# scroll-tech/scroll-prover

Hardware: AMD Instinct MI355X
Metric: BN254 MSM G1-adds/sec at k=26 (higher is better)
Workload: dtype u32 (9x29-bit limbs of 254-bit Montgomery integers; v_mad_u64_u32); 1 GPU; BN254 G1 Pippenger MSM, 2^26 uniform random scalars x synthetic SRS points, inputs resident in HBM; point-range shards over 1 GPU(s), RCCL all-gather of 96-B partials; log_n=26, window_bits=22, windows=12, parallelism=point-range x1, one rank per GPU, srs_window_tables=True

## Files before the change

### scroll-prover_amd/csrc/fp29.hpp

```cpp
#pragma once
#include "fp.hpp"

namespace zk {

struct fe29_t { uint32_t l[9]; };
constexpr uint32_t M29 = (1u << 29) - 1;

struct Fq29P {
  static constexpr uint32_t INV = 0x4866389u;
  ZK_HD static constexpr uint32_t mod(int i) { constexpr uint32_t m[9] = {0x187cfd47u, 0x10460b6u, 0x1c72a34fu, 0x2d522d0u, 0x1585d978u, 0x2db40c0u, 0xa6e141u, 0xe5c2634u, 0x30644eu}; return m[i]; }
  ZK_HD static constexpr uint32_t one(int i) { constexpr uint32_t m[9] = {0x157ccc21u, 0x141c2758u, 0x185230d3u, 0x14c0419u, 0xaa36fb9u, 0x1d4240ceu, 0x11d54c07u, 0x52ac7a8u, 0xdc836u}; return m[i]; }
  ZK_HD static constexpr uint32_t r256(int i) { constexpr uint32_t m[9] = {0x58f0d9du, 0x1aea1c6eu, 0x11c2cf74u, 0x11d651ebu, 0x1462c0a7u, 0x11b7bc3cu, 0x1cbd99bau, 0x183340fbu, 0xe0a77u}; return m[i]; }
  ZK_HD static constexpr uint32_t fat29_4p(int i) { constexpr uint32_t m[9] = {0x21f3f51cu, 0x241182dau, 0x31ca8d3bu, 0x2b548b42u, 0x361765dfu, 0x2b6d0301u, 0x229b8503u, 0x397098cfu, 0xc19138u}; return m[i]; }
  ZK_HD static constexpr uint32_t fat30_8p(int i) { constexpr uint32_t m[9] = {0x43e7ea38u, 0x482305b4u, 0x43951a76u, 0x56a91685u, 0x4c2ecbbeu, 0x56da0603u, 0x45370a06u, 0x52e1319eu, 0x1832271u}; return m[i]; }
  ZK_HD static constexpr uint32_t fat30_16p(int i) { constexpr uint32_t m[9] = {0x47cfd470u, 0x50460b6au, 0x472a34eeu, 0x4d522d0cu, 0x585d977fu, 0x4db40c08u, 0x4a6e140fu, 0x45c2633eu, 0x30644e5u}; return m[i]; }
};
struct Fr29P {
  static constexpr uint32_t INV = 0xfffffffu;
  ZK_HD static constexpr uint32_t mod(int i) { constexpr uint32_t m[9] = {0x10000001u, 0x1f0fac9fu, 0xe5c2450u, 0x7d090f3u, 0x1585d283u, 0x2db40c0u, 0xa6e141u, 0xe5c2634u, 0x30644eu}; return m[i]; }
  ZK_HD static constexpr uint32_t one(int i) { constexpr uint32_t m[9] = {0xfffff57u, 0x1ea70ab4u, 0x52c068bu, 0x17504f49u, 0xaa8075bu, 0x1d4240ceu, 0x11d54c07u, 0x52ac7a8u, 0xdc836u}; return m[i]; }
  ZK_HD static constexpr uint32_t r256(int i) { constexpr uint32_t m[9] = {0xffffffbu, 0x4b1a0e2u, 0x18334a6bu, 0x18ed2b3eu, 0x1462e36fu, 0x11b7bc3cu, 0x1cbd99bau, 0x183340fbu, 0xe0a77u}; return m[i]; }
  ZK_HD static constexpr uint32_t fat29_4p(int i) { constexpr uint32_t m[9] = {0x20000004u, 0x3c3eb27du, 0x39709142u, 0x3f4243ccu, 0x36174a0bu, 0x2b6d0301u, 0x229b8503u, 0x397098cfu, 0xc19138u}; return m[i]; }
  ZK_HD static constexpr uint32_t fat30_8p(int i) { constexpr uint32_t m[9] = {0x40000008u, 0x587d64fau, 0x52e12285u, 0x5e848799u, 0x4c2e9417u, 0x56da0603u, 0x45370a06u, 0x52e1319eu, 0x1832271u}; return m[i]; }
  ZK_HD static constexpr uint32_t fat30_16p(int i) { constexpr uint32_t m[9] = {0x40000010u, 0x50fac9f6u, 0x45c2450du, 0x5d090f35u, 0x585d2831u, 0x4db40c08u, 0x4a6e140fu, 0x45c2633eu, 0x30644e5u}; return m[i]; }
};

#if defined(__HIP_DEVICE_COMPILE__)
#include "fp29_asm_gen.inc"
#endif

template <class P> struct Fp29 {
  ZK_HD static fe29_t zero() { fe29_t r; for (int i = 0; i < 9; i++) r.l[i] = 0; return r; }
  ZK_HD static fe29_t one() { fe29_t r; for (int i = 0; i < 9; i++) r.l[i] = P::one(i); return r; }

  ZK_HD static fe29_t mul(const fe29_t &a, const fe29_t &b) {
    uint64_t acc = 0; uint32_t m[9]; fe29_t r;
#pragma unroll
    for (int k = 0; k < 9; k++) {
#pragma unroll
      for (int i = 0; i <= k; i++) acc += (uint64_t)a.l[i] * b.l[k - i];
#pragma unroll
      for (int i = 0; i < k; i++) acc += (uint64_t)m[i] * P::mod(k - i);
      m[k] = ((uint32_t)acc * P::INV) & M29;
      acc += (uint64_t)m[k] * P::mod(0);
      acc >>= 29;
    }
#pragma unroll
    for (int k = 9; k < 17; k++) {
#pragma unroll
      for (int i = k - 8; i < 9; i++) acc += (uint64_t)a.l[i] * b.l[k - i];
#pragma unroll
      for (int i = k - 8; i < 9; i++) acc += (uint64_t)m[i] * P::mod(k - i);
      r.l[k - 9] = (uint32_t)acc & M29;
      acc >>= 29;
    }
    r.l[8] = (uint32_t)acc;
    return r;
  }
  ZK_HD static fe29_t sqr(const fe29_t &a) {
    uint64_t acc = 0; uint32_t m[9]; fe29_t r;
    uint32_t a2[9];
#pragma unroll
    for (int i = 0; i < 9; i++) a2[i] = a.l[i] << 1;
#pragma unroll
    for (int k = 0; k < 9; k++) {
#pragma unroll
      for (int i = 0; 2 * i < k; i++) acc += (uint64_t)a.l[i] * a2[k - i];
      if ((k & 1) == 0) acc += (uint64_t)a.l[k / 2] * a.l[k / 2];
#pragma unroll
      for (int i = 0; i < k; i++) acc += (uint64_t)m[i] * P::mod(k - i);
      m[k] = ((uint32_t)acc * P::INV) & M29;
      acc += (uint64_t)m[k] * P::mod(0);
      acc >>= 29;
    }
#pragma unroll
    for (int k = 9; k < 17; k++) {
#pragma unroll
      for (int i = k - 8; 2 * i < k; i++) acc += (uint64_t)a.l[i] * a2[k - i];
      if ((k & 1) == 0) acc += (uint64_t)a.l[k / 2] * a.l[k / 2];
#pragma unroll
      for (int i = k - 8; i < 9; i++) acc += (uint64_t)m[i] * P::mod(k - i);
      r.l[k - 9] = (uint32_t)acc & M29;
      acc >>= 29;
    }
    r.l[8] = (uint32_t)acc;
    return r;
  }
  ZK_HD static fe29_t mul_sub(const fe29_t &a, const fe29_t &b, const fe29_t &c, const fe29_t &d) {
    int64_t acc = 0; uint32_t m[9]; fe29_t r;
    int32_t nc[9];
#pragma unroll
    for (int i = 0; i < 9; i++) nc[i] = -(int32_t)c.l[i];
#pragma unroll
    for (int k = 0; k < 9; k++) {
#pragma unroll
      for (int i = 0; i <= k; i++) { acc += (int64_t)(int32_t)a.l[i] * (int32_t)b.l[k - i]; acc += (int64_t)nc[i] * (int32_t)d.l[k - i]; }
#pragma unroll
      for (int i = 0; i < k; i++) acc += (int64_t)(int32_t)m[i] * (int32_t)P::mod(k - i);
      m[k] = ((uint32_t)acc * P::INV) & M29;
      acc += (int64_t)(int32_t)m[k] * (int32_t)P::mod(0);
      acc >>= 29;
    }
#pragma unroll
    for (int k = 9; k < 17; k++) {
#pragma unroll
      for (int i = k - 8; i < 9; i++) { acc += (int64_t)(int32_t)a.l[i] * (int32_t)b.l[k - i]; acc += (int64_t)nc[i] * (int32_t)d.l[k - i]; }
#pragma unroll
      for (int i = k - 8; i < 9; i++) acc += (int64_t)(int32_t)m[i] * (int32_t)P::mod(k - i);
      r.l[k - 9] = ((uint32_t)acc & M29) + P::mod(k - 9);
      acc >>= 29;
    }
    r.l[8] = (uint32_t)((int32_t)acc + (int32_t)P::mod(8));
    return r;
  }
  ZK_HD static fe29_t mul_c(const fe29_t &a, const fe29_t &b) {
#if defined(__HIP_DEVICE_COMPILE__)
    uint64_t acc = 0, co; uint32_t m[9]; fe29_t r;
    ZK_FP29_MUL_COLUMNS
    (void)co;
    return r;
#else
    return mul(a, b);
#endif
  }
  ZK_HD static fe29_t sqr_c(const fe29_t &a) {
#if defined(__HIP_DEVICE_COMPILE__)
    uint64_t acc = 0, co; uint32_t m[9]; fe29_t r;
    uint32_t a2[9];
#pragma unroll
    for (int i = 0; i < 9; i++) a2[i] = a.l[i] << 1;
    ZK_FP29_SQR_COLUMNS
    (void)co;
    return r;
#else
    return sqr(a);
#endif
  }
  ZK_HD static fe29_t mul_sub_c(const fe29_t &a, const fe29_t &b, const fe29_t &c, const fe29_t &d) {
#if defined(__HIP_DEVICE_COMPILE__)
    int64_t acc = 0; uint64_t co; uint32_t m[9]; fe29_t r;
    int32_t nc[9];
#pragma unroll
    for (int i = 0; i < 9; i++) nc[i] = -(int32_t)c.l[i];
    ZK_FP29_MULSUB_COLUMNS
    (void)co;
    return r;
#else
    return mul_sub(a, b, c, d);
#endif
  }
  ZK_HD static fe29_t carry(const fe29_t &a) {
    fe29_t r; r.l[0] = a.l[0] & M29;
#pragma unroll
    for (int i = 1; i < 8; i++) r.l[i] = (a.l[i] & M29) + (a.l[i - 1] >> 29);
    r.l[8] = a.l[8] + (a.l[7] >> 29);
    return r;
  }
  ZK_HD static fe29_t add(const fe29_t &a, const fe29_t &b) { fe29_t r; for (int i = 0; i < 9; i++) r.l[i] = a.l[i] + b.l[i]; return r; }
  ZK_HD static fe29_t sub4(const fe29_t &a, const fe29_t &b) {
    fe29_t r;
#pragma unroll
    for (int i = 0; i < 9; i++) r.l[i] = a.l[i] + P::fat29_4p(i) - b.l[i];
    return carry(r);
  }
  ZK_HD static fe29_t sub4_lazy(const fe29_t &a, const fe29_t &b) {
    fe29_t r;
#pragma unroll
    for (int i = 0; i < 9; i++) r.l[i] = a.l[i] + P::fat29_4p(i) - b.l[i];
    return r;
  }
  ZK_HD static fe29_t sub8(const fe29_t &a, const fe29_t &b) {
    fe29_t r;
#pragma unroll
    for (int i = 0; i < 9; i++) r.l[i] = a.l[i] + P::fat30_8p(i) - b.l[i];
    return carry(r);
  }
  ZK_HD static fe29_t sub4_8(const fe29_t &a, const fe29_t &b, const fe29_t &c) {
    fe29_t r;
#pragma unroll
    for (int i = 0; i < 9; i++) r.l[i] = a.l[i] + (P::fat29_4p(i) + P::fat30_8p(i)) - b.l[i] - c.l[i];
    return carry(r);
  }
  ZK_HD static fe29_t sub16(const fe29_t &a, const fe29_t &b) {
    fe29_t r;
#pragma unroll
    for (int i = 0; i < 9; i++) r.l[i] = a.l[i] + P::fat30_16p(i) - b.l[i];
    return carry(r);
  }
  ZK_HD static fe29_t dbl(const fe29_t &a) { fe29_t r; for (int i = 0; i < 9; i++) r.l[i] = a.l[i] << 1; return r; }

  ZK_HD static fe29_t normalise(const fe29_t &a) {
    fe29_t r; uint32_t c = 0;
#pragma unroll
    for (int i = 0; i < 8; i++) { uint32_t v = a.l[i] + c; r.l[i] = v & M29; c = v >> 29; }
    r.l[8] = a.l[8] + c;
    return r;
  }
  ZK_HD static fe29_t cond_sub_p(const fe29_t &a) {
    fe29_t d; uint32_t borrow = 0;
#pragma unroll
    for (int i = 0; i < 9; i++) { uint32_t v = a.l[i] - P::mod(i) - borrow; borrow = v >> 31; d.l[i] = (i < 8) ? (v & M29) : v; }
    fe29_t r;
#pragma unroll
    for (int i = 0; i < 9; i++) r.l[i] = borrow ? a.l[i] : d.l[i];
    return r;
  }
  ZK_HD static fe29_t reduce_small(const fe29_t &v) {
    const uint32_t q = (uint32_t)(((uint64_t)(v.l[8] >> 12) * 0x15291u) >> 26);
    fe29_t r; int64_t c = 0;
#pragma unroll
    for (int i = 0; i < 9; i++) { c += (int64_t)v.l[i] - (int64_t)((uint64_t)q * P::mod(i)); r.l[i] = (i < 8) ? ((uint32_t)c & M29) : (uint32_t)c; c >>= 29; }
    return r;
  }
  ZK_HD static bool is_zero_tight(const fe29_t &a) {
    if (a.l[0] != 0 && a.l[0] != P::mod(0)) return false;
    uint32_t z = 0, q = 0;
#pragma unroll
    for (int i = 0; i < 9; i++) { z |= a.l[i]; q |= a.l[i] ^ P::mod(i); }
    return z == 0 || q == 0;
  }
  ZK_HD static fe29_t from_sat(const fe_t &s) {
    fe29_t r;
    r.l[0] = (s.l[0] << 5) & M29;
#pragma unroll
    for (int i = 1; i < 9; i++) {
      const int bit = 29 * i - 5, w = bit >> 5, sh = bit & 31;
      uint32_t v = s.l[w] >> sh;
      if (sh > 3 && w + 1 < 8) v |= s.l[w + 1] << (32 - sh);
      r.l[i] = v & M29;
    }
    return r;
  }
  ZK_HD static fe29_t from_sat_plain(const fe_t &s) {
    fe29_t r;
#pragma unroll
    for (int i = 0; i < 9; i++) {
      const int bit = 29 * i, w = bit >> 5, sh = bit & 31;
      uint32_t v = s.l[w] >> sh;
      if (sh > 3 && w + 1 < 8) v |= s.l[w + 1] << (32 - sh);
      r.l[i] = v & M29;
    }
    return r;
  }
  ZK_HD static fe_t to_sat_plain(const fe29_t &a) {
    fe_t s;
#pragma unroll
    for (int w = 0; w < 8; w++) {
      const int bit = 32 * w, i = bit / 29, sh = bit - 29 * i;
      uint64_t v = (uint64_t)a.l[i] >> sh;
      v |= (uint64_t)a.l[i + 1] << (29 - sh);
      if (i + 2 < 9) v |= (uint64_t)a.l[i + 2] << (58 - sh);
      s.l[w] = (uint32_t)v;
    }
    return s;
  }
  ZK_HD static fe_t to_sat(const fe29_t &a) {
    fe29_t c; for (int i = 0; i < 9; i++) c.l[i] = P::r256(i);
    fe29_t t = cond_sub_p(normalise(mul(a, c)));
    return to_sat_plain(t);
  }
};

using Fq29 = Fp29<Fq29P>;
using Fr29 = Fp29<Fr29P>;

}
```

### scroll-prover_amd/csrc/g1_29.hpp

```cpp
#pragma once
#include "fp29.hpp"
#include "g1.hpp"

namespace zk {

struct g1_xyzz29_t { fe29_t x, y, zz, zzz; };

ZK_HD g1_xyzz29_t g1_xyzz29_identity() { g1_xyzz29_t r; r.x = Fq29::zero(); r.y = Fq29::zero(); r.zz = Fq29::zero(); r.zzz = Fq29::zero(); return r; }
ZK_HD bool g1_xyzz29_is_identity(const g1_xyzz29_t &p) { uint32_t o = 0; for (int i = 0; i < 9; i++) o |= p.zz.l[i]; return o == 0; }

ZK_HD fe29_t fq29_neg_loaded(const fe29_t &y) {
  constexpr uint32_t c[9] = {0x3f3f51c0u, 0x21182dafu, 0x3ca8d3c1u, 0x3548b437u, 0x21765e04u, 0x36d0302au, 0x29b85044u, 0x37098d00u, 0xc19139bu};
  fe29_t r;
#pragma unroll
  for (int i = 0; i < 9; i++) r.l[i] = c[i] - y.l[i];
  return r;
}

ZK_HD g1_xyzz29_t g1_xyzz29_dbl_affine(const fe29_t &xt, const fe29_t &yt) {
  const fe29_t U = Fq29::dbl(yt);
  const fe29_t V = Fq29::sqr_c(U), W = Fq29::mul_c(U, V), S = Fq29::mul_c(xt, V);
  const fe29_t xx = Fq29::sqr_c(xt);
  const fe29_t M = Fq29::carry(Fq29::add(Fq29::dbl(xx), xx));
  g1_xyzz29_t r;
  r.x = Fq29::sub8(Fq29::sqr_c(M), Fq29::dbl(S));
  const fe29_t t = Fq29::sub16(S, r.x);
  r.y = Fq29::sub4(Fq29::mul_c(M, t), Fq29::mul_c(W, yt));
  r.zz = V; r.zzz = W;
  return r;
}

ZK_HD bool g1_affine_is_identity_x(const g1_affine_t &q) { return Fq::is_zero(q.x); }
ZK_HD fe29_t fq29_negx(const fe29_t &x) { return Fq29::sub16(Fq29::zero(), x); }
ZK_HD void g1_xyzz29_negx_to_plain(g1_xyzz29_t &acc) { if (!g1_xyzz29_is_identity(acc)) acc.x = fq29_negx(acc.x); }

ZK_HD void g1_xyzz29_madd_core(g1_xyzz29_t &acc, const fe29_t &x2, const fe29_t &y2, bool y2_needs_normalise);
ZK_HD void g1_xyzz29_madd(g1_xyzz29_t &acc, const g1_affine_t &q, bool negate) {
  if (g1_affine_is_identity_x(q)) return;
  const fe29_t x2 = Fq29::from_sat(q.x);
  fe29_t y2 = Fq29::from_sat(q.y);
  if (negate) y2 = fq29_neg_loaded(y2);
  g1_xyzz29_madd_core(acc, x2, y2, negate);
}
ZK_HD void g1_xyzz29_madd_core(g1_xyzz29_t &acc, const fe29_t &x2, const fe29_t &y2, bool y2_needs_normalise) {
  if (g1_xyzz29_is_identity(acc)) {
    acc.x = Fq29::reduce_small(x2); acc.y = Fq29::reduce_small(y2_needs_normalise ? Fq29::normalise(y2) : y2);
    acc.x = Fq29::sub4(Fq29::zero(), acc.x);
    acc.zz = Fq29::one(); acc.zzz = Fq29::one();
    return;
  }
  const fe29_t U2 = Fq29::mul_c(x2, acc.zz), S2 = Fq29::mul_c(y2, acc.zzz);
  const fe29_t Pd = Fq29::add(U2, acc.x);
  const fe29_t Rd = Fq29::sub8(S2, acc.y);
  const fe29_t PP = Fq29::sqr_c(Pd);
  const fe29_t ZZ3 = Fq29::mul_c(acc.zz, PP);
  if (Fq29::is_zero_tight(ZZ3)) {
    const fe29_t one = Fq29::one();
    if (Fq29::is_zero_tight(Fq29::mul(Rd, one))) { acc = g1_xyzz29_dbl_affine(Fq29::mul(x2, one), Fq29::mul(y2, one)); acc.x = fq29_negx(acc.x); }
    else acc = g1_xyzz29_identity();
    return;
  }
  const fe29_t PPP = Fq29::mul_c(Pd, PP);
  const fe29_t Qn = Fq29::mul_c(acc.x, PP);
  const fe29_t xn3 = Fq29::sub4_8(PPP, Fq29::sqr_c(Rd), Fq29::dbl(Qn));
  const fe29_t T = Fq29::sub4_lazy(xn3, Qn);
  const fe29_t Y3 = Fq29::mul_sub_c(Rd, T, acc.y, PPP);
  acc.x = xn3; acc.y = Y3; acc.zz = ZZ3; acc.zzz = Fq29::mul_c(acc.zzz, PPP);
}

ZK_HD g1_xyzz29_t g1_xyzz29_dbl(const g1_xyzz29_t &a) {
  if (g1_xyzz29_is_identity(a)) return a;
  const fe29_t xt = Fq29::reduce_small(Fq29::normalise(a.x));
  const fe29_t yc = Fq29::carry(a.y);
  const fe29_t U = Fq29::dbl(yc);
  const fe29_t V = Fq29::sqr_c(U), W = Fq29::mul_c(U, V), S = Fq29::mul_c(xt, V);
  const fe29_t xx = Fq29::sqr_c(xt);
  const fe29_t M = Fq29::carry(Fq29::add(Fq29::dbl(xx), xx));
  g1_xyzz29_t r;
  r.x = Fq29::sub8(Fq29::sqr_c(M), Fq29::dbl(S));
  const fe29_t t = Fq29::sub16(S, r.x);
  r.y = Fq29::sub4(Fq29::mul_c(M, t), Fq29::mul_c(W, yc));
  r.zz = Fq29::mul_c(V, a.zz); r.zzz = Fq29::mul_c(W, a.zzz);
  return r;
}

ZK_HD void g1_xyzz29_add(g1_xyzz29_t &acc, const g1_xyzz29_t &q) {
  if (g1_xyzz29_is_identity(q)) return;
  if (g1_xyzz29_is_identity(acc)) { acc = q; return; }
  const fe29_t U1 = Fq29::mul_c(acc.x, q.zz), S1 = Fq29::mul_c(acc.y, q.zzz);
  const fe29_t U2 = Fq29::mul_c(q.x, acc.zz), S2 = Fq29::mul_c(q.y, acc.zzz);
  const fe29_t Pd = Fq29::sub4(U2, U1);
  const fe29_t Rd = Fq29::sub4(S2, S1);
  const fe29_t PP = Fq29::sqr_c(Pd);
  const fe29_t ZZt = Fq29::mul_c(acc.zz, PP);
  if (Fq29::is_zero_tight(ZZt)) {
    if (Fq29::is_zero_tight(Fq29::mul_c(Rd, Fq29::one()))) acc = g1_xyzz29_dbl(acc);
    else acc = g1_xyzz29_identity();
    return;
  }
  const fe29_t PPP = Fq29::mul_c(Pd, PP);
  const fe29_t Q = Fq29::mul_c(U1, PP);
  const fe29_t X3 = Fq29::sub4_8(Fq29::sqr_c(Rd), PPP, Fq29::dbl(Q));
  const fe29_t Y3 = Fq29::mul_sub_c(Rd, Fq29::sub16(Q, X3), S1, PPP);
  acc.x = X3; acc.y = Y3;
  acc.zz = Fq29::mul_c(ZZt, q.zz); acc.zzz = Fq29::mul_c(Fq29::mul_c(acc.zzz, PPP), q.zzz);
}

ZK_HD g1_xyzz_t g1_xyzz29_to_sat(const g1_xyzz29_t &a) {
  g1_xyzz_t r;
  if (g1_xyzz29_is_identity(a)) return g1_xyzz_identity();
  r.x = Fq29::to_sat(a.x); r.y = Fq29::to_sat(a.y); r.zz = Fq29::to_sat(a.zz); r.zzz = Fq29::to_sat(a.zzz);
  return r;
}

}
```

### scroll-prover_amd/csrc/lib_common.hpp

```cpp
#pragma once
#include <hip/hip_runtime.h>
#include <stdio.h>
#include <stdlib.h>
#include <string.h>
#include <algorithm>
#include <atomic>
#include <chrono>
#include <map>
#include <memory>
#include <mutex>
#include <string>
#include <thread>
#include <condition_variable>
#include <unordered_map>
#include <vector>

#include "../../include/mi355zk.h"
#include "fp.hpp"
#include "g1.hpp"
#include "g1_29.hpp"
#include "ntt_types.hpp"
#include "ws_layout.hpp"
#include "knobs.hpp"

namespace mi355 {
using namespace zk;
using mi355zk::WsLayout;

extern thread_local std::string g_err;
int fail(int code, const std::string &msg);

#define HIPCHK(expr)                                                                                                     \
  do {                                                                                                                   \
    hipError_t _e = (expr);                                                                                              \
    if (_e != hipSuccess) {                                                                                              \
      char _b[512]; snprintf(_b, sizeof _b, "%s failed: %s (%s:%d)", #expr, hipGetErrorString(_e), __FILE__, __LINE__);  \
      (void)hipGetLastError();                                                                                           \
      return ::mi355::fail(_e == hipErrorOutOfMemory ? MI355_EOOM : MI355_EHIP, _b);                                     \
    }                                                                                                                    \
  } while (0)
#define CHK(expr) do { int _r = (expr); if (_r != MI355_OK) return _r; } while (0)

struct Shard { int slot = 0; uint64_t lo = 0, n = 0; g1_affine_t *dev = nullptr; bool owned = false; };
void free_shards(std::vector<Shard> &sh);
struct SrsMem { std::vector<Shard> sh; ~SrsMem() { free_shards(sh); } };
struct SrsTables { std::vector<g1_affine_t *> pre; std::vector<uint64_t> stride; std::vector<int> slot; int c = 0, w = 0; ~SrsTables(); };
struct Srs { uint64_t n = 0; std::shared_ptr<SrsMem> mem; std::shared_ptr<SrsTables> tab; };
struct Buf { void *p = nullptr; size_t cap = 0; };
struct NttPlan {
  uint32_t log_n = 0, levels = 0, log_m[3] = {0, 0, 0};
  uint32_t split[2] = {0, 0};
  uint32_t direct2[2] = {0, 0};
  std::map<std::string, Tw29> scaled;
  struct CosetTw { Tw29 in, s2d; };
  std::map<std::string, CosetTw> coset;
  Tw29 tw29_m[3] = {}, tw29_s_lo[2] = {}, tw29_s_hi[2] = {};
  std::vector<void *> owned;
};
struct Prof { double ms = 0; uint64_t launches = 0; };

struct MsmSlot { int id = 0; hipEvent_t sorted = nullptr, acc_done = nullptr, red_done = nullptr; bool used = false; };

struct Span { std::string name; hipEvent_t a, b; };
struct Ctx : mi355zk::Knobs {
  bool inited = false;
  int slot = 0;
  int device = -1;
  hipDeviceProp_t prop;
  hipStream_t own_stream = nullptr, stream = nullptr;
  hipStream_t aux_stream[2] = {nullptr, nullptr};
  hipStream_t copy_stream = nullptr;
  MsmSlot msm_slot[2];
  hipEvent_t ev_fork = nullptr;
  hipEvent_t ev_xchg = nullptr;
  hipEvent_t ev_xchg2 = nullptr;
  hipEvent_t ev_copy[4] = {};
  hipEvent_t ev_up[8] = {}; uint32_t up_next = 0;
  hipEvent_t ev_up_fork = nullptr;
  void *comm = nullptr;
  std::vector<const fe_t *> polys_stage;
  uint32_t msm_chunk_min_log = 23;
  int last_chunks = 1;
  std::map<std::string, Buf> ws;
  std::map<std::string, NttPlan> ntt_plans;
  g1_affine_t *fixed_base_table = nullptr;
  bool profiling = false;
  std::vector<Span> spans;
  std::map<std::string, Prof> prof;
  int last_c = 0, last_w = 0; uint64_t last_entries = 0; bool last_shared = false; int last_host_slices = 1;
};
enum : unsigned { SYNC_COMPUTE = 1, SYNC_AUX = 2, SYNC_COPY = 4 };
struct CtxStream { hipStream_t *s; unsigned kind; };
inline std::vector<CtxStream> ctx_streams(Ctx &c) { return {{&c.own_stream, SYNC_COMPUTE}, {&c.aux_stream[0], SYNC_AUX}, {&c.aux_stream[1], SYNC_AUX}, {&c.copy_stream, SYNC_COPY}}; }
inline std::vector<hipEvent_t *> ctx_events(Ctx &c) {
  std::vector<hipEvent_t *> v = {&c.ev_fork, &c.ev_xchg, &c.ev_xchg2, &c.ev_up_fork};
  for (auto &m : c.msm_slot) { v.push_back(&m.sorted); v.push_back(&m.acc_done); v.push_back(&m.red_done); }
  for (auto &e : c.ev_copy) v.push_back(&e);
  for (auto &e : c.ev_up) v.push_back(&e);
  return v;
}
hipError_t sync_streams(Ctx &c, unsigned which);

constexpr int MAX_DEV = 16;
extern std::mutex g_ctx_mu[MAX_DEV];
extern std::mutex g_upload_mu[MAX_DEV];
extern Ctx g_ctx[MAX_DEV];
extern int g_ndev;
extern bool g_dup_devices;
extern bool g_peer_ok[MAX_DEV][MAX_DEV];
extern mi355zk::ProcessKnobs g_proc;
extern thread_local Ctx *g_cur;
#define g (*::mi355::g_cur)
extern std::unordered_map<uint64_t, Srs> &g_srs;
extern uint64_t g_next_handle;
extern int g_last_devices; extern const char *g_last_exchange;

struct DevGuard {
  std::unique_lock<std::mutex> lk;
  explicit DevGuard(int slot) : lk(g_ctx_mu[slot]) {}
};
struct AllGuard {
  std::unique_lock<std::mutex> lk[MAX_DEV];
  AllGuard() { for (int i = 0; i < MAX_DEV; i++) lk[i] = std::unique_lock<std::mutex>(g_ctx_mu[i]); }
};
struct MsmGuard {
  std::unique_lock<std::mutex> lk[MAX_DEV];
  MsmGuard() { lk[0] = std::unique_lock<std::mutex>(g_ctx_mu[0]); for (int i = 1; i < g_ndev && i < MAX_DEV; i++) lk[i] = std::unique_lock<std::mutex>(g_ctx_mu[i]); }
};

struct PoolBlock {
  void *p = nullptr; int slot = 0;
  PoolBlock() = default;
  PoolBlock(const PoolBlock &) = delete; PoolBlock &operator=(const PoolBlock &) = delete;
  ~PoolBlock() { if (p) (void)mi355_buf_free(p); }
  int alloc(uint64_t bytes, int slot_) { slot = slot_; return mi355_buf_alloc(bytes, slot_, &p); }
  char *at(uint64_t off) const { return (char *)p + off; }
  int upload(uint64_t off, const void *src_host, uint64_t bytes);
};

struct MsmOpts { bool normalise = true; int force_c = 0; bool no_tables = false; };
extern thread_local MsmOpts t_opts;

inline void use_ctx(int slot) { g_cur = &g_ctx[slot]; }
int bind_ctx(int slot);
int need_init(int slot = 0);
inline int PoolBlock::upload(uint64_t off, const void *src_host, uint64_t bytes) { CHK(mi355_buf_upload(at(off), src_host, bytes)); return need_init(slot); }

struct CallTrace {
  const char *what; uint64_t n; double bytes_per_unit; std::chrono::steady_clock::time_point t0;
  CallTrace(const char *w, uint64_t n_, double bpu) : what(w), n(n_), bytes_per_unit(bpu), t0(std::chrono::steady_clock::now()) {}
  void done(const char *extra = "") {
    if (!g.trace) return;
    (void)hipStreamSynchronize(g.stream);
    const double ms = std::chrono::duration<double, std::milli>(std::chrono::steady_clock::now() - t0).count();
    fprintf(stderr, "[mi355zk] %s n=%llu %.3f ms %.2f M units/s %.1f GB/s algorithmic%s\n", what, (unsigned long long)n, ms, n / ms / 1e3, n * bytes_per_unit / ms / 1e6, extra);
  }
};

int ws_get(const char *role, size_t bytes, void **out);
int dev_malloc(void **out, size_t bytes, const char *what);

struct Scope {
  bool on; hipEvent_t a = nullptr, b = nullptr; std::string name; hipStream_t st;
  Scope(const char *n, hipStream_t s = nullptr) : on(g.profiling), name(n), st(s ? s : g.stream) { if (on) { (void)hipEventCreate(&a); (void)hipEventCreate(&b); (void)hipEventRecord(a, st); } }
  void close() { if (on) { (void)hipEventRecord(b, st); g.spans.push_back({name, a, b}); on = false; } }
  ~Scope() { close(); }
};
void resolve_spans();
inline int finish_async() { if (g.profiling) resolve_spans(); return MI355_OK; }

inline uint32_t ceil_div(uint64_t a, uint64_t b) { return (uint32_t)((a + b - 1) / b); }
inline uint32_t log2_ceil(uint64_t n) { uint32_t l = 0; while ((1ull << l) < n) l++; return l; }

struct Roctx { int state = 0; int (*push)(const char *) = nullptr; int (*pop)() = nullptr; };
extern Roctx g_roctx;
void roctx_bind();
struct ApiRange {
  bool on;
  explicit ApiRange(const char *name) : on(false) { if (g_roctx.state == 0) roctx_bind(); if (g_roctx.state == 2) { g_roctx.push(name); on = true; } }
  ~ApiRange() { if (on) g_roctx.pop(); }
};
template <class F> int guarded(F body, const char *who = __builtin_FUNCTION()) {
  ApiRange range(who);
  try { return body(); }
  catch (const std::bad_alloc &) { return fail(MI355_EOOM, "host allocation failed"); }
  catch (const std::exception &e) { return fail(MI355_EHIP, std::string("unexpected host exception: ") + e.what()); }
  catch (...) { return fail(MI355_EHIP, "unexpected host exception"); }
}

struct Rccl {
  void *lib = nullptr;
  int (*CommInitAll)(void **, int, const int *) = nullptr;
  int (*CommDestroy)(void *) = nullptr;
  int (*AllGather)(const void *, void *, size_t, int, void *, hipStream_t) = nullptr;
  int (*GroupStart)() = nullptr;
  int (*GroupEnd)() = nullptr;
  const char *(*GetErrorString)(int) = nullptr;
};
extern Rccl g_rccl;
int rccl_fail(const char *what, int rc);

std::vector<Shard> plan_shards(uint64_t n);
int srs_find(uint64_t handle, Srs **out, const char *who);
uint64_t srs_insert(const Srs &s);
int srs_alloc(SrsMem &mem, uint64_t n);
int srs_scatter_from_primary(SrsMem &mem, const g1_affine_t *src_dev, uint64_t n, bool alias_shard0);
int srs_gather_to_primary(const Srs &sr, uint64_t n, const g1_affine_t **out);

int slot_of(const void *dev_ptr, bool touch = true);
int buf_check_range(const void *dev_ptr, uint64_t bytes, const char *who);
int common_slot(std::initializer_list<const void *> ptrs, int *slot_out, const char *who);
int common_slot(const void *const *ptrs, size_t count, bool touch, int *slot_out, const char *who);
int pick_replica_slot();

int msm_tu_init_device();
int ntt_tu_init_device();
int aux_tu_init_device();
int launch_pow_table(fe_t *out, const fe_t &base, uint64_t step, uint32_t count);
int launch_g1_decompress(const void *bytes_dev, void *affine_out_dev, uint64_t n, uint64_t base, unsigned long long *err_dev);
bool g2_decode_host(const uint8_t in[64], void *g2affine_out);
constexpr int MSM_SCALAR_BITS = 255, MSM_MAX_C = 24;
double msm_cost(uint64_t n, int c, bool shared);

inline int check_ntt_args(const void *data, uint32_t log_n, const void *omega) {
  if (!data || !omega) return fail(MI355_EBADARG, "ntt: null pointer");
  if (log_n > 28) return fail(MI355_EBADARG, "ntt: log_n > 28");
  return MI355_OK;
}
struct NttHostArgs { uint32_t log_n; const void *omega; const void *divisor; };
inline int with_host_io(void *data_host, size_t in_bytes, size_t out_bytes, size_t dev_bytes, const char *role, int (*body)(void *dev, void *ud), void *ud) {
  void *dev; CHK(ws_get(role, dev_bytes, &dev));
  HIPCHK(hipMemcpyAsync(dev, data_host, in_bytes, hipMemcpyHostToDevice, g.stream));
  CHK(body(dev, ud));
  HIPCHK(hipMemcpyAsync(data_host, dev, out_bytes, hipMemcpyDeviceToHost, g.stream));
  HIPCHK(hipStreamSynchronize(g.stream));
  resolve_spans();
  return MI355_OK;
}

}
```

### scroll-prover_amd/csrc/lib_msm.hip

```cpp
#define ZK_FRSCAN_DEVICE_ONLY 1
#include "msm.hpp"
#define ZK_G2_DEVICE_ONLY 1
#include "msm_g2.hpp"
#include "msm_seg.hpp"
#include "lib_common.hpp"

namespace mi355 {

static_assert(sizeof(fe_t) == 32 && sizeof(g1_affine_t) == 64 && sizeof(g1_jac_t) == 96, "ABI element sizes");
static_assert(sizeof(g1_xyzz_t) == 128 && sizeof(g1_xyzz29_t) == 144, "device record sizes (workspace layout, 16-byte vector accesses)");

int msm_tu_init_device() {
  HIPCHK(hipFuncSetAttribute((const void *)k_sort_l1_scatter_split<24>, hipFuncAttributeMaxDynamicSharedMemorySize, 160 * 1024));
  HIPCHK(hipFuncSetAttribute((const void *)k_sort_l1_scatter_split<16>, hipFuncAttributeMaxDynamicSharedMemorySize, 160 * 1024));
  HIPCHK(hipFuncSetAttribute((const void *)k_sort_l1_scatter_split<8>, hipFuncAttributeMaxDynamicSharedMemorySize, 160 * 1024));
  HIPCHK(hipFuncSetAttribute((const void *)k_sort_l2_scatter_split<16>, hipFuncAttributeMaxDynamicSharedMemorySize, 160 * 1024));
  HIPCHK(hipFuncSetAttribute((const void *)k_sort_l2_scatter_split<8>, hipFuncAttributeMaxDynamicSharedMemorySize, 160 * 1024));
  return MI355_OK;
}

double msm_cost(uint64_t n, int c, bool shared) { const double W = (MSM_SCALAR_BITS + c - 1) / c, nb = (double)(1ull << (c - 1)); return 1.18 * W * (double)n + 8.2 * nb * (shared ? 1.0 : W) + (shared ? 0.0 : 3.0e7); }

int choose_c(uint64_t n) {
  if (t_opts.force_c) return t_opts.force_c;
  double best = 1e300; int best_c = 8;
  for (int c = 4; c <= (int)g_proc.msm_auto_max_c; c++) {
    const double W = (MSM_SCALAR_BITS + c - 1) / c, nb = (double)(1ull << (c - 1));
    if (W * nb * sizeof(g1_xyzz29_t) > 6.0e9) continue;
    const double cost = msm_cost(n, c, false);
    if (cost < best) { best = cost; best_c = c; }
  }
  return best_c;
}

struct PreTable { const g1_affine_t *table = nullptr; uint64_t row_stride = 0; int c = 0, w = 0; };
const PreTable *pre_advance(const PreTable *pre, uint64_t lo, PreTable &store) {
  if (!pre) return nullptr;
  store = *pre; if (store.table) store.table += lo;
  return &store;
}

struct MsmShape { bool shared; uint32_t c, W, fb, cb_bits, regions; uint64_t emax, nbuckets; };
int msm_shape(uint64_t n, uint32_t M, const PreTable *pre, MsmShape &o, const MsmShape *forced = nullptr) {
  if (forced) { o.c = forced->c; o.shared = forced->shared; }
  else {
    o.c = (uint32_t)choose_c(n);
    o.shared = pre && pre->table && !t_opts.force_c && !t_opts.no_tables && msm_cost(n, pre->c, true) <= msm_cost(n, (int)o.c, false) && ((uint64_t)pre->w << log2_ceil(n)) < (1ull << 31);
    if (o.shared) o.c = (uint32_t)pre->c;
  }
  o.W = (MSM_SCALAR_BITS + o.c - 1) / o.c;
  o.emax = (uint64_t)M * n * o.W;
  const uint32_t kb = o.c - 1; uint32_t fb = kb < g.sort_fb ? kb : g.sort_fb; if (kb - fb > 11) fb = kb - 11;
  o.fb = fb; o.cb_bits = kb - fb;
  const uint64_t sets = (uint64_t)M * (o.shared ? 1 : o.W);
  o.nbuckets = sets << kb;
  const uint64_t regions = sets << o.cb_bits; o.regions = (uint32_t)std::min<uint64_t>(regions, 0xffffffffu);
  if (o.emax >= (1ull << 32)) return fail(MI355_EBADARG, "msm: n * windows must be < 2^32");
  if (o.nbuckets >= (1ull << 31)) return fail(MI355_EBADARG, "msm: too many buckets (split the batch)");
  if (regions * 4 > 48 * 1024) return fail(MI355_EBADARG, "msm: batch too large for the coarse histogram (split the batch)");
  if (o.fb > 12 || (1u << o.cb_bits) > SORT_MAX_BINS) return fail(MI355_EBADARG, "msm: window bits out of range for the sorter");
  return MI355_OK;
}

template <class G> bool msm_batch_must_split(uint64_t n, uint32_t M, const PreTable *pre) {
  MsmShape sh;
  return msm_shape(n, M, pre, sh) != MI355_OK || sh.emax > (1ull << 29) || sh.nbuckets * sizeof(typename G::rec_t) > (8ull << 30);
}

struct Roles {
  const char *prefix; std::string sfx;
  template <class T> int get(const char *name, size_t bytes, T *&ptr) const { return ws_get((std::string(prefix) + name + sfx).c_str(), bytes, (void **)&ptr); }
};

int msm_stage_polys(const fe_t *const *polys_host, uint32_t M, const Roles &ws, hipStream_t s, PolyPtrs &inl, const fe_t **&polys_dev) {
  if (M <= 8) { for (uint32_t m = 0; m < M; m++) inl.p[m] = polys_host[m]; return MI355_OK; }
  CHK(ws.get("polys", (size_t)M * sizeof(void *), polys_dev));
  g.polys_stage.assign(polys_host, polys_host + M);
  HIPCHK(hipMemcpyAsync(polys_dev, g.polys_stage.data(), (size_t)M * sizeof(void *), hipMemcpyHostToDevice, s));
  HIPCHK(hipStreamSynchronize(s));
  return MI355_OK;
}

struct AccPlan { uint32_t seg, blocks, tn; };
AccPlan msm_acc_plan(uint64_t emax) {
  const uint64_t want_threads = (uint64_t)g.prop.multiProcessorCount * 256 * g.seg_factor;
  uint64_t seg = (emax + want_threads - 1) / want_threads; if (seg < 16) seg = 16; if (seg > 4096) seg = 4096;
  const uint32_t blocks = ceil_div(ceil_div(emax, seg), 256);
  return {(uint32_t)seg, blocks, blocks * 256};
}
uint32_t msm_seg_arg(uint32_t seg, uint32_t fill_pct) { return seg | (std::min(g.seg_min, seg) << 13) | ((fill_pct / 2) << 26); }
MsmPlan msm_plan(const MsmShape &sh, uint64_t n, uint32_t M, uint32_t seg) {
  MsmPlan P; P.n = (uint32_t)n; P.c = sh.c; P.windows = sh.W; P.nb = 1u << (sh.c - 1); P.seg = seg; P.batch = M;
  return P;
}

template <class G, class F> void with_lanes(bool quad, F &&launch) {
  if constexpr (G::QUAD) { if (quad) { launch(std::integral_constant<int, 4>{}); return; } }
  launch(std::integral_constant<int, 1>{});
}

template <class G> int msm_segfix_levels(const int32_t *part_id, const typename G::rec_t *part, uint32_t tn, typename G::rec_t *buckets, hipStream_t s, const Roles &ws) {
  using rec_t = typename G::rec_t;
  uint32_t N = 2 * tn; const uint32_t waves1 = ceil_div(N, 64);
  const size_t cap = (size_t)2 * waves1 + (size_t)waves1 / 8 + 512;
  int32_t *lv_ids; rec_t *lv_recs;
  CHK(ws.get("segfix_ids", cap * 4, lv_ids)); CHK(ws.get("segfix_recs", cap * sizeof(rec_t), lv_recs));
  const int32_t *cur_ids = part_id; const rec_t *cur_recs = part; size_t used = 0;
  while (N > 64) {
    const uint32_t waves = ceil_div(N, 64);
    hipLaunchKernelGGL(k_msm_segfix<G>, dim3(ceil_div(N, 256)), dim3(256), 0, s, cur_ids, cur_recs, N, buckets, lv_ids + used, lv_recs + used, 0);
    cur_ids = lv_ids + used; cur_recs = lv_recs + used; used += (size_t)2 * waves; N = 2 * waves;
  }
  hipLaunchKernelGGL(k_msm_segfix<G>, dim3(1), dim3(64), 0, s, cur_ids, cur_recs, N, buckets, (int32_t *)nullptr, (rec_t *)nullptr, 1);
  return MI355_OK;
}

template <class G> int msm_reduce_tail(const MsmShape &sh, uint32_t M, const typename G::rec_t *buckets, typename G::out_t *out_dev, bool normalise, hipStream_t s, const Roles &ws) {
  using rec_t = typename G::rec_t;
  const uint32_t nb = 1u << (sh.c - 1), wpp = sh.shared ? 1 : sh.W, sets = M * wpp;
  uint32_t chunk = 64; while (chunk > nb) chunk >>= 1;
  while (chunk > g.reduce_min_chunk && (uint64_t)(nb / chunk) * sets < g.reduce_chains) chunk >>= 1;
  const uint32_t chunks_per_set = nb / chunk, nchunks = chunks_per_set * sets;
  rec_t *chunk_out, *tree_a, *tree_b, *window_sums;
  CHK(ws.get("chunk_out", (size_t)nchunks * sizeof(rec_t), chunk_out));
  { const size_t lvl = (size_t)ceil_div(chunks_per_set, 64 * TREE_PER_THREAD) * sets + 1;
    CHK(ws.get("tree_a", lvl * sizeof(rec_t), tree_a)); CHK(ws.get("tree_b", lvl * sizeof(rec_t), tree_b)); }
  CHK(ws.get("window_sums", (size_t)sets * sizeof(rec_t), window_sums));
  with_lanes<G>(nchunks <= g.tail_coop_max && (g.tail_coop_mask & 2u), [&](auto q) {
    constexpr int Q = decltype(q)::value;
    hipLaunchKernelGGL((k_msm_bucket_reduce<G, Q>), dim3(ceil_div((uint64_t)nchunks * Q, 128)), dim3(128), 0, s, buckets, chunk_out, nb, sets, chunk);
  });
  const rec_t *cur = chunk_out; uint32_t cnt = chunks_per_set; rec_t *bufs[2] = {tree_a, tree_b}; int which = 0;
  while (true) {
    const bool coop = G::QUAD && (uint64_t)cnt * sets <= g.tail_coop_max && (g.tail_coop_mask & 4u);
    const uint32_t outn = ceil_div(cnt, (coop ? 64u : 256u) * TREE_PER_THREAD);
    rec_t *dst = outn == 1 ? window_sums : bufs[which];
    with_lanes<G>(coop, [&](auto q) { hipLaunchKernelGGL((k_msm_tree_sum<G, decltype(q)::value>), dim3(outn, sets), dim3(256), 0, s, cur, cnt, dst, outn); });
    if (outn == 1) break;
    cur = dst; cnt = outn; which ^= 1;
  }
  with_lanes<G>(g.tail_coop_max && (g.tail_coop_mask & 8u), [&](auto q) {
    hipLaunchKernelGGL((k_msm_final<G, decltype(q)::value>), dim3(M), dim3(64), 0, s, (const rec_t *)window_sums, wpp, sh.shared ? 0u : sh.c, out_dev, normalise ? 1 : 0);
  });
  HIPCHK(hipGetLastError());
  return MI355_OK;
}

int msm_sort_stage(const PolyPtrs &inl, const fe_t *const *polys_dev, uint32_t M, uint64_t n, const MsmShape &sh, const MsmPlan &P, uint32_t *offsets, uint32_t *sorted,
                   hipStream_t s, bool g2 = false) {
  const bool shared = sh.shared;
  const uint64_t emax = sh.emax;
  const uint32_t nbuckets = (uint32_t)sh.nbuckets;
  SortPlan S; S.n = P.n; S.windows = M * P.windows; S.wpp = P.windows; S.nb = P.nb;
  S.fb = sh.fb; S.cb_bits = sh.cb_bits;
  S.shared = shared ? 1 : 0; S.nshift = log2_ceil(n);
  S.regions = sh.regions;
  S.t1 = g.sort_t1;
  if (g.sort_split == 1 && S.t1 == 16384 && (1u << S.cb_bits) <= 1024 && emax >= (1ull << 24)) S.t1 = 24576;
  S.t2 = g.sort_t2 ? g.sort_t2 : (emax >= (1ull << 27) && S.fb <= 11 ? 16384 : 8192);
  const uint32_t tiles1 = ceil_div(n, S.t1), l2_tiles_max = ceil_div(emax, S.t2) + S.regions + 8;
  const uint32_t vwindows = M * P.windows;

  uint32_t *enc, *hist, *cursor, *scan_sums, *coarse_hist, *coarse_off, *coarse_cursor, *tile_start;
  CHK(ws_get("msm.digits", emax * 4, (void **)&enc));
  uint32_t *pairs_lo = nullptr; uint16_t *pairs_hi = nullptr;
  CHK(ws_get("msm.pairs_lo", emax * 4 + 64, (void **)&pairs_lo)); CHK(ws_get("msm.pairs_hi", emax * 2 + 64, (void **)&pairs_hi));
  CHK(ws_get("msm.hist", ((size_t)nbuckets + 1) * 4, (void **)&hist));
  CHK(ws_get("msm.cursor", ((size_t)nbuckets + 1) * 4, (void **)&cursor));
  CHK(ws_get("msm.coarse_hist", ((size_t)S.regions + 1) * 4, (void **)&coarse_hist));
  CHK(ws_get("msm.coarse_off", ((size_t)S.regions + 1) * 4, (void **)&coarse_off));
  CHK(ws_get("msm.coarse_cursor", ((size_t)S.regions + 1) * 4, (void **)&coarse_cursor));
  CHK(ws_get("msm.tile_start", ((size_t)S.regions + 1) * 4, (void **)&tile_start));
  const uint32_t scan_n = nbuckets + 1, scan_blocks = ceil_div(scan_n, SCAN_BLOCK * SCAN_ITEMS);
  const uint32_t cscan_n = S.regions + 1, cscan_blocks = ceil_div(cscan_n, SCAN_BLOCK * SCAN_ITEMS);
  CHK(ws_get("msm.scan_sums", (size_t)(scan_blocks + cscan_blocks) * 4, (void **)&scan_sums));
  const int grid_stream = g.prop.multiProcessorCount * 8;
  {
    Scope sc(g2 ? "msm_g2_digits" : "msm_digits", s);
    HIPCHK(hipMemsetAsync(coarse_hist, 0, ((size_t)S.regions + 1) * 4, s));
    const dim3 dgrid(grid_stream / M > 0 ? grid_stream / M : 1, M);
    if (g2) hipLaunchKernelGGL(k_msm_digits<false>, dgrid, dim3(256), (size_t)S.regions * 4, s, inl, polys_dev, enc, P, coarse_hist, S.fb, S.cb_bits, S.shared);
    else hipLaunchKernelGGL(k_msm_digits<true>, dgrid, dim3(256), (size_t)S.regions * 4, s, inl, polys_dev, enc, P, coarse_hist, S.fb, S.cb_bits, S.shared);
  }
  {
    Scope sc(g2 ? "msm_g2_sort" : "msm_sort", s);
    HIPCHK(hipMemsetAsync(hist, 0, ((size_t)nbuckets + 1) * 4, s));
    hipLaunchKernelGGL(k_scan_partial, dim3(cscan_blocks), dim3(SCAN_BLOCK), 0, s, coarse_hist, scan_sums + scan_blocks, cscan_n);
    hipLaunchKernelGGL(k_scan_block_sums, dim3(1), dim3(SCAN_BLOCK), 0, s, scan_sums + scan_blocks, cscan_blocks);
    hipLaunchKernelGGL(k_scan_final, dim3(cscan_blocks), dim3(SCAN_BLOCK), 0, s, coarse_hist, scan_sums + scan_blocks, coarse_off, coarse_cursor, cscan_n);
    {
      Scope s1(g2 ? "g2_sort_l1" : "sort_l1", s);
      const uint32_t CBp = ((1u << S.cb_bits) + 1) & ~1u;
      const size_t lds1 = (size_t)(3 * CBp + 32 + SORT_SPLIT_TMAX) * 4 + (size_t)S.t1 * 6;
      if (S.t1 == 24576) hipLaunchKernelGGL(k_sort_l1_scatter_split<24>, dim3(tiles1 * vwindows), dim3(1024), lds1, s, enc, coarse_cursor, pairs_lo, pairs_hi, S);
      else if (S.t1 == 16384) hipLaunchKernelGGL(k_sort_l1_scatter_split<16>, dim3(tiles1 * vwindows), dim3(1024), lds1, s, enc, coarse_cursor, pairs_lo, pairs_hi, S);
      else hipLaunchKernelGGL(k_sort_l1_scatter_split<8>, dim3(tiles1 * vwindows), dim3(1024), lds1, s, enc, coarse_cursor, pairs_lo, pairs_hi, S);
    }
    hipLaunchKernelGGL(k_sort_tile_prefix, dim3(1), dim3(SCAN_BLOCK), 0, s, coarse_off, tile_start, S);
    { Scope s2(g2 ? "g2_sort_hist" : "sort_hist", s);
    hipLaunchKernelGGL(k_sort_l2_hist_split, dim3(l2_tiles_max), dim3(256), 0, s, (const uint16_t *)pairs_hi, coarse_off, tile_start, hist, S); }
    hipLaunchKernelGGL(k_scan_partial, dim3(scan_blocks), dim3(SCAN_BLOCK), 0, s, hist, scan_sums, scan_n);
    hipLaunchKernelGGL(k_scan_block_sums, dim3(1), dim3(SCAN_BLOCK), 0, s, scan_sums, scan_blocks);
    hipLaunchKernelGGL(k_scan_final, dim3(scan_blocks), dim3(SCAN_BLOCK), 0, s, hist, scan_sums, offsets, cursor, scan_n);
    {
      Scope s3(g2 ? "g2_sort_l2" : "sort_l2", s);
      const size_t lds2 = (size_t)(3 * (1u << S.fb) + 32) * 4 + (size_t)S.t2 * 6;
      if (S.t2 == 8192) hipLaunchKernelGGL(k_sort_l2_scatter_split<8>, dim3(l2_tiles_max), dim3(1024), lds2, s, (const uint32_t *)pairs_lo, (const uint16_t *)pairs_hi, coarse_off, tile_start, cursor, sorted, S);
      else hipLaunchKernelGGL(k_sort_l2_scatter_split<16>, dim3(l2_tiles_max), dim3(1024), lds2, s, (const uint32_t *)pairs_lo, (const uint16_t *)pairs_hi, coarse_off, tile_start, cursor, sorted, S);
    }
  }
  return MI355_OK;
}

struct MsmStreams { hipStream_t a, b, c; };

int msm_enqueue(const g1_affine_t *bases, const PolyPtrs &inl, const fe_t *const *polys_dev, uint32_t M, uint64_t n, g1_jac_t *out_dev, const PreTable *pre, MsmSlot &slot,
                const MsmStreams &st, bool normalise, const MsmShape *forced = nullptr, uint32_t set_index = 0, uint32_t set_count = 1, bool skip_tail = false) {
  const bool piped = st.a != st.b;
  const Roles ws{G1Ops::ROLE, slot.id ? "#" + std::to_string(slot.id) : std::string()};
  MsmShape sh; CHK(msm_shape(n, M, pre, sh, forced));
  const bool shared = sh.shared;
  if (shared) bases = pre->table;
  const uint64_t emax = sh.emax;
  const AccPlan ap = msm_acc_plan(emax);
  const MsmPlan P = msm_plan(sh, n, M, ap.seg);
  const bool segfix = g.fixup_mode == 1 || (g.fixup_mode == 2 && (uint32_t)sh.nbuckets >= (1u << 19) && (uint64_t)P.seg * sh.nbuckets >= emax);
  const uint32_t seg_arg = msm_seg_arg(P.seg, segfix ? g.seg_fill_segfix : g.seg_fill);
  const uint32_t nbuckets = (uint32_t)sh.nbuckets;
  const uint32_t acc_blocks = ap.blocks, tn = ap.tn;
  uint32_t *offsets, *sorted;
  g1_xyzz29_t *buckets, *part; int32_t *part_id;
  CHK(ws.get("offsets", ((size_t)nbuckets + 1) * 4, offsets));
  CHK(ws.get("sorted", emax * 4, sorted));
  CHK(ws.get("buckets", (size_t)nbuckets * set_count * sizeof(g1_xyzz29_t), buckets));
  buckets += (size_t)nbuckets * set_index;
  CHK(ws.get("part", (size_t)tn * 2 * sizeof(g1_xyzz29_t), part));
  CHK(ws.get("part_id", (size_t)tn * 2 * 4, part_id));
  const uint32_t big_cap = tn / g.fixup_serial_max + 2;
  uint32_t *big_list; CHK(ws.get("big_list", ((size_t)big_cap * 3 + 1) * 4, big_list));
  uint32_t *big_count = big_list + (size_t)big_cap * 3;
  const uint32_t huge_cap = tn / FIXUP_HUGE_MIN + 2;
  uint32_t *huge_list, *huge_count; g1_xyzz29_t *huge_part;
  CHK(ws.get("huge_list", ((size_t)huge_cap * 3 + 1) * 4, huge_list)); huge_count = huge_list + (size_t)huge_cap * 3;
  CHK(ws.get("huge_part", (size_t)huge_cap * FIXUP_SLICES * sizeof(g1_xyzz29_t), huge_part));

  {
    hipStream_t s = st.a;
    if (piped && slot.used) { HIPCHK(hipStreamWaitEvent(s, slot.acc_done, 0)); HIPCHK(hipStreamWaitEvent(s, slot.red_done, 0)); }
    CHK(msm_sort_stage(inl, polys_dev, M, n, sh, P, offsets, sorted, s));
    if (piped) { HIPCHK(hipEventRecord(slot.sorted, s)); HIPCHK(hipStreamWaitEvent(st.b, slot.sorted, 0)); }
  }
  {
    hipStream_t s = st.b;
    if (piped && slot.used) HIPCHK(hipStreamWaitEvent(s, slot.red_done, 0));
    {
      Scope sc("msm_accumulate", s);
      HIPCHK(hipMemsetAsync(buckets, 0, (size_t)nbuckets * sizeof(g1_xyzz29_t), s));
      hipLaunchKernelGGL(k_msm_accumulate, dim3(acc_blocks), dim3(256), 0, s, bases, sorted, offsets, nbuckets, buckets, part, part_id, seg_arg, log2_ceil(n), shared ? pre->row_stride : (uint64_t)0);
    }
    if (piped) { HIPCHK(hipEventRecord(slot.acc_done, s)); HIPCHK(hipStreamWaitEvent(st.c, slot.acc_done, 0)); }
  }
  {
    hipStream_t s = st.c;
    Scope sc("msm_reduce", s);
    HIPCHK(hipMemsetAsync(big_count, 0, 4, s));
    HIPCHK(hipMemsetAsync(huge_count, 0, 4, s));
    if (segfix) CHK(msm_segfix_levels<G1Ops>(part_id, part, tn, buckets, s, ws));
    else {
      auto fixup = [&](auto kernel, uint64_t threads) {
        hipLaunchKernelGGL(kernel, dim3(ceil_div(threads, 256)), dim3(256), 0, s, offsets, nbuckets, buckets, part, part_id, seg_arg, tn, big_list, big_count, big_cap, huge_list, huge_count, huge_cap, g.fixup_serial_max, g.fixup_huge_min);
      };
      if ((uint64_t)nbuckets * 4 <= g.tail_coop_max && (g.tail_coop_mask & 1u)) fixup(k_msm_fixup<4, 4>, (uint64_t)nbuckets * 16);
      else if (nbuckets <= (1u << g.fixup_lanes_max_log)) fixup(k_msm_fixup<4, 1>, (uint64_t)nbuckets * 4);
      else fixup(k_msm_fixup<1, 1>, nbuckets);
      hipLaunchKernelGGL(k_msm_fixup_big, dim3(big_cap), dim3(256), 0, s, buckets, part, part_id, big_list, big_count);
      hipLaunchKernelGGL(k_msm_fixup_huge, dim3(huge_cap * FIXUP_SLICES), dim3(256), 0, s, part, part_id, huge_list, huge_count, huge_part, huge_cap);
      hipLaunchKernelGGL(k_msm_fixup_huge_fold, dim3(huge_cap), dim3(64), 0, s, buckets, huge_list, huge_count, (const g1_xyzz29_t *)huge_part);
    }
    if (!skip_tail) CHK(msm_reduce_tail<G1Ops>(sh, M, buckets, out_dev, normalise, s, ws));
  }
  if (piped) HIPCHK(hipEventRecord(slot.red_done, st.c));
  slot.used = true;
  HIPCHK(hipGetLastError());
  g.last_c = (int)P.c; g.last_w = (int)P.windows; g.last_entries += emax; g.last_shared = shared;
  return MI355_OK;
}

uint32_t msm_chunks_for(uint32_t M, uint64_t n) {
  if (g.msm_chunks <= 1 || M != 1 || n < (1ull << g.msm_chunk_min_log)) return 1;
  uint32_t k = g.msm_chunks;
  while (k > 1 && n / k < ((1ull << g.msm_chunk_min_log) >> 2)) k--;
  return k;
}

int msm_deliver(CallTrace &tr, const g1_jac_t *out_dev, uint32_t M, void *out_host, void *out_dev_user, hipStream_t s, const char *what, uint32_t count) {
  if (out_dev_user) {
    HIPCHK(hipMemcpyAsync(out_dev_user, out_dev, (size_t)M * sizeof(g1_jac_t), hipMemcpyDeviceToDevice, s));
    if (g.profiling) resolve_spans();
    tr.done(" (device result)");
    return MI355_OK;
  }
  HIPCHK(hipMemcpyAsync(out_host, out_dev, (size_t)M * sizeof(g1_jac_t), hipMemcpyDeviceToHost, s));
  HIPCHK(hipStreamSynchronize(s));
  resolve_spans();
  { char buf[64]; snprintf(buf, sizeof buf, " %s=%u c=%d W=%d", what, count, g.last_c, g.last_w); tr.done(buf); }
  return MI355_OK;
}

int msm_batch_impl(const g1_affine_t *bases, const fe_t *const *polys_host, uint32_t M, uint64_t n, void *out_host, const PreTable *pre, void *out_dev_user = nullptr, bool accumulate_plan = false) {
  if (M == 0) return MI355_OK;
  if (n == 0) {
    if (out_dev_user) { HIPCHK(hipMemsetAsync(out_dev_user, 0, (size_t)M * sizeof(g1_jac_t), g.stream)); return MI355_OK; }
    memset(out_host, 0, (size_t)M * sizeof(g1_jac_t)); return MI355_OK;
  }
  if (n >= (1ull << 31)) return fail(MI355_EBADARG, "msm: n must be < 2^31");
  if (M > 1 && msm_batch_must_split<G1Ops>(n, M, pre)) {
    const uint32_t h = M / 2;
    CHK(msm_batch_impl(bases, polys_host, h, n, out_host, pre, out_dev_user, accumulate_plan));
    return msm_batch_impl(bases, polys_host + h, M - h, n, out_host ? (char *)out_host + (size_t)h * sizeof(g1_jac_t) : nullptr, pre,
                          out_dev_user ? (char *)out_dev_user + (size_t)h * sizeof(g1_jac_t) : nullptr, true);
  }
  const uint32_t K = msm_chunks_for(M, n);
  if (!accumulate_plan) { g.last_entries = 0; g.last_host_slices = 1; }
  CallTrace tr("msm_g1", (uint64_t)M * n, 96.0);
  g1_jac_t *out_dev; const fe_t **polys_dev = nullptr;
  CHK(ws_get("msm.out", (size_t)(K + 1) * M * sizeof(g1_jac_t), (void **)&out_dev));
  hipStream_t s = g.stream;
  Scope total("msm_total", s);
  PolyPtrs inl{};
  if (K == 1) {
    CHK(msm_stage_polys(polys_host, M, Roles{G1Ops::ROLE, ""}, s, inl, polys_dev));
    MsmStreams st{s, s, s};
    CHK(msm_enqueue(bases, inl, polys_dev, M, n, out_dev, pre, g.msm_slot[0], st, t_opts.normalise));
  } else {
    std::vector<uint64_t> lo(K + 1);
    for (uint32_t k = 0; k <= K; k++) lo[k] = n * k / K;
    HIPCHK(hipEventRecord(g.ev_fork, s));
    HIPCHK(hipStreamWaitEvent(g.aux_stream[0], g.ev_fork, 0)); HIPCHK(hipStreamWaitEvent(g.aux_stream[1], g.ev_fork, 0));
    MsmStreams st{g.aux_stream[0], s, g.aux_stream[1]};
    for (uint32_t k = 0; k < K; k++) {
      PreTable pk; const PreTable *pp = pre_advance(pre, lo[k], pk);
      inl.p[0] = polys_host[0] + lo[k];
      CHK(msm_enqueue(bases + lo[k], inl, nullptr, M, lo[k + 1] - lo[k], out_dev + (size_t)(k + 1) * M, pp, g.msm_slot[k & 1], st, false));
    }
    HIPCHK(hipStreamWaitEvent(s, g.msm_slot[0].red_done, 0)); HIPCHK(hipStreamWaitEvent(s, g.msm_slot[1].red_done, 0));
    HIPCHK(hipEventRecord(g.ev_fork, st.a)); HIPCHK(hipStreamWaitEvent(s, g.ev_fork, 0));
    hipLaunchKernelGGL(k_g1_sum_strided, dim3(M), dim3(64), 0, s, out_dev + M, K, M, out_dev, t_opts.normalise ? 1 : 0);
  }
  HIPCHK(hipGetLastError());
  total.close();
  g.msm_slot[0].used = g.msm_slot[1].used = false;
  g.last_chunks = (int)K;
  return msm_deliver(tr, out_dev, M, out_host, out_dev_user, s, "batch", M);
}

int msm_host_single(const g1_affine_t *bases, const fe_t *const *polys_host, uint32_t M, uint64_t n, void *out_host, const PreTable *pre, void *out_dev_user = nullptr) {
  fe_t *sc; CHK(ws_get("io.scalars", (size_t)M * n * sizeof(fe_t), (void **)&sc));
  hipStream_t s = g.stream;
  std::vector<uint64_t> cut;
  if (M == 1 && n >= (1ull << g.host_slice_min_log) && g.host_chunks > 1) {
    double w = 1.0, tot = 0; std::vector<double> ws;
    const double first = 1.0 / 16.0;
    for (double rem = 1.0; rem > 1e-9 && ws.size() + 1 < g.host_chunks;) { const double take = std::min(rem, first * w); ws.push_back(take); rem -= take; w *= 1.7; tot += take; }
    if (tot < 1.0 - 1e-9) ws.push_back(1.0 - tot);
    cut.push_back(0); double acc = 0;
    const uint64_t align = n >= (1ull << 20) ? ~1023ull : ~0ull;
    for (size_t i = 0; i + 1 < ws.size(); i++) { acc += ws[i]; const uint64_t c = std::min<uint64_t>(n, (uint64_t)(acc * (double)n) & align); if (c > cut.back() && c < n) cut.push_back(c); }
    cut.push_back(n);
  }
  uint32_t K = cut.empty() ? 1 : (uint32_t)cut.size() - 1;
  uint64_t biggest = 0; for (uint32_t k = 0; k < K && !cut.empty(); k++) biggest = std::max(biggest, cut[k + 1] - cut[k]);
  MsmShape shape;
  if (K > 1 && (msm_shape(biggest, 1, pre, shape) != MI355_OK || shape.nbuckets * K * sizeof(g1_xyzz29_t) > (8ull << 30))) K = 1;
  if (K <= 1) {
    std::vector<const fe_t *> ptrs(M);
    for (uint32_t m = 0; m < M; m++) { ptrs[m] = sc + (size_t)m * n; HIPCHK(hipMemcpyAsync(sc + (size_t)m * n, polys_host[m], n * sizeof(fe_t), hipMemcpyHostToDevice, s)); }
    return msm_batch_impl(bases, ptrs.data(), M, n, out_host, pre, out_dev_user);
  }
  g.last_entries = 0;
  CallTrace tr("msm_g1_host", n, 96.0);
  g1_jac_t *out_dev; CHK(ws_get("msm.out", 2 * sizeof(g1_jac_t), (void **)&out_dev));
  Scope total("msm_total", s);
  HIPCHK(hipEventRecord(g.ev_fork, s)); HIPCHK(hipStreamWaitEvent(g.copy_stream, g.ev_fork, 0));
  PolyPtrs inl{};
  MsmStreams st{s, s, s};
  for (uint32_t k = 0; k < K; k++) {
    const uint64_t lo = cut[k], hi = cut[k + 1];
    HIPCHK(hipMemcpyAsync(sc + lo, polys_host[0] + lo, (hi - lo) * sizeof(fe_t), hipMemcpyHostToDevice, g.copy_stream));
    HIPCHK(hipEventRecord(g.ev_copy[k & 3], g.copy_stream));
    HIPCHK(hipStreamWaitEvent(s, g.ev_copy[k & 3], 0));
    PreTable pk; const PreTable *pp = pre_advance(pre, lo, pk);
    inl.p[0] = sc + lo;
    CHK(msm_enqueue(bases + lo, inl, nullptr, 1, hi - lo, out_dev, pp, g.msm_slot[0], st, t_opts.normalise, &shape, k, K, true));
  }
  g.msm_slot[0].used = false;
  g1_xyzz29_t *buckets; CHK(ws_get("msm.buckets", (size_t)shape.nbuckets * K * sizeof(g1_xyzz29_t), (void **)&buckets));
  {
    Scope sc2("msm_reduce", s);
    hipLaunchKernelGGL(k_msm_bucket_fold, dim3(ceil_div(shape.nbuckets, 256)), dim3(256), 0, s, buckets, (uint32_t)shape.nbuckets, K);
    CHK(msm_reduce_tail<G1Ops>(shape, 1, buckets, out_dev, t_opts.normalise, s, Roles{G1Ops::ROLE, ""}));
  }
  total.close();
  g.last_chunks = (int)K; g.last_host_slices = (int)K;
  return msm_deliver(tr, out_dev, 1, out_host, out_dev_user, s, "host slices", K);
}

static int msm_g2_impl(const g2_affine_t *bases, const fe_t *const *polys, uint32_t M, uint64_t n, void *out_host, bool accumulate_plan = false) {
  if (M == 0) return MI355_OK;
  if (n == 0) { memset(out_host, 0, (size_t)M * sizeof(g2_affine_t)); return MI355_OK; }
  if (n >= (1ull << 31)) return fail(MI355_EBADARG, "msm_g2: n must be < 2^31");
  if (M > 1 && msm_batch_must_split<G2Ops>(n, M, nullptr)) {
    const uint32_t h = M / 2;
    CHK(msm_g2_impl(bases, polys, h, n, out_host, accumulate_plan));
    return msm_g2_impl(bases, polys + h, M - h, n, (char *)out_host + (size_t)h * sizeof(g2_affine_t), true);
  }
  MsmShape sh; CHK(msm_shape(n, M, nullptr, sh));
  if (!accumulate_plan) { g.last_entries = 0; g.last_host_slices = 1; }
  CallTrace tr("msm_g2", (uint64_t)M * n, 160.0);
  hipStream_t s = g.stream;
  Scope total("msm_g2_total", s);
  const Roles ws{G2Ops::ROLE, ""};
  const AccPlan ap = msm_acc_plan(sh.emax);
  const MsmPlan P = msm_plan(sh, n, M, ap.seg);
  const uint32_t nbuckets = (uint32_t)sh.nbuckets;
  PolyPtrs inl{}; const fe_t **polys_dev = nullptr;
  CHK(msm_stage_polys(polys, M, ws, s, inl, polys_dev));
  uint32_t *offsets, *sorted; g2_xyzz_t *buckets, *part; int32_t *part_id;
  CHK(ws.get("offsets", ((size_t)nbuckets + 1) * 4, offsets));
  CHK(ws.get("sorted", sh.emax * 4, sorted));
  CHK(ws.get("buckets", (size_t)nbuckets * sizeof(g2_xyzz_t), buckets));
  CHK(ws.get("part", (size_t)ap.tn * 2 * sizeof(g2_xyzz_t), part));
  CHK(ws.get("part_id", (size_t)ap.tn * 2 * 4, part_id));
  CHK(msm_sort_stage(inl, polys_dev, M, n, sh, P, offsets, sorted, s, true));
  {
    Scope sc("msm_g2_accumulate", s);
    HIPCHK(hipMemsetAsync(buckets, 0, (size_t)nbuckets * sizeof(g2_xyzz_t), s));
    hipLaunchKernelGGL(k_msm_g2_accumulate, dim3(ap.blocks), dim3(256), 0, s, bases, sorted, offsets, nbuckets, buckets, part, part_id, msm_seg_arg(P.seg, 100));
  }
  {
    Scope sc("msm_g2_fixup", s);
    CHK(msm_segfix_levels<G2Ops>(part_id, part, ap.tn, buckets, s, ws));
  }
  g2_affine_t *out_dev; CHK(ws.get("out", (size_t)M * sizeof(g2_affine_t), out_dev));
  {
    Scope sc("msm_g2_reduce", s);
    CHK(msm_reduce_tail<G2Ops>(sh, M, buckets, out_dev, true, s, ws));
  }
  total.close();
  HIPCHK(hipMemcpyAsync(out_host, out_dev, (size_t)M * sizeof(g2_affine_t), hipMemcpyDeviceToHost, s));
  HIPCHK(hipStreamSynchronize(s));
  resolve_spans();
  g.last_c = (int)P.c; g.last_w = (int)P.windows; g.last_entries += sh.emax; g.last_shared = false; g.last_chunks = 1;
  { char buf[64]; snprintf(buf, sizeof buf, " batch=%u c=%d W=%d", M, g.last_c, g.last_w); tr.done(buf); }
  return MI355_OK;
}
static int msm_g2_run(const g2_affine_t *bases, const fe_t *const *polys, uint32_t M, uint64_t n, void *out_host) {
  if (n) {
    uint32_t *bad; CHK(ws_get("msm2.validate", 4, (void **)&bad));
    Scope sc("msm_g2_validate", g.stream);
    HIPCHK(hipMemsetAsync(bad, 0xff, 4, g.stream));
    const uint32_t blocks = std::min<uint64_t>(ceil_div(n, 256), (uint64_t)g.prop.multiProcessorCount * 8);
    hipLaunchKernelGGL(k_msm_g2_validate, dim3(blocks), dim3(256), 0, g.stream, bases, n, g2_twist_b(), bad);
    HIPCHK(hipGetLastError());
    uint32_t first_bad = 0xffffffffu;
    HIPCHK(hipMemcpyAsync(&first_bad, bad, 4, hipMemcpyDeviceToHost, g.stream));
    HIPCHK(hipStreamSynchronize(g.stream));
    sc.close();
    if (first_bad != 0xffffffffu) return fail(MI355_EBADARG, "msm_g2: base " + std::to_string(first_bad) + " is not on the twist y^2 = x^3 + 3 / (9 + u)");
  }
  g_last_devices = 1; g_last_exchange = "none";
  return msm_g2_impl(bases, polys, M, n, out_host);
}

}

using namespace mi355;

extern "C" {

static int stream_file_to_device(FILE *f, void *dev, size_t bytes, void *pinned[2], size_t chunk) {
  hipEvent_t ev[2] = {nullptr, nullptr};
  for (int i = 0; i < 2; i++) { HIPCHK(hipEventCreateWithFlags(&ev[i], hipEventDisableTiming)); HIPCHK(hipEventRecord(ev[i], g.stream)); }
  size_t done = 0; int which = 0; int rc = MI355_OK;
  while (done < bytes && rc == MI355_OK) {
    const size_t len = std::min(chunk, bytes - done);
    if (hipEventSynchronize(ev[which]) != hipSuccess) { rc = fail(MI355_EHIP, "srs_load_params_file: event wait failed"); break; }
    if (fread(pinned[which], 1, len, f) != len) { rc = fail(MI355_EBADARG, "srs_load_params_file: short read"); break; }
    if (hipMemcpyAsync((char *)dev + done, pinned[which], len, hipMemcpyHostToDevice, g.stream) != hipSuccess || hipEventRecord(ev[which], g.stream) != hipSuccess) { (void)hipGetLastError(); rc = fail(MI355_EHIP, "srs_load_params_file: copy failed"); break; }
    done += len; which ^= 1;
  }
  (void)hipStreamSynchronize(g.stream);
  for (int i = 0; i < 2; i++) (void)hipEventDestroy(ev[i]);
  return rc;
}
static int stream_processed_to_shard(FILE *f, const Shard &sh, void *pinned[2], size_t chunk_pts, unsigned long long *bad_out) {
  PoolBlock stage; CHK(stage.alloc(2 * chunk_pts * 32, sh.slot));
  struct Side {
    hipStream_t cs = nullptr; hipEvent_t copied[2] = {nullptr, nullptr}, used[2] = {nullptr, nullptr};
    ~Side() {
      if (cs) (void)hipStreamSynchronize(cs);
      (void)hipStreamSynchronize(g.stream);
      for (int i = 0; i < 2; i++) { if (copied[i]) (void)hipEventDestroy(copied[i]); if (used[i]) (void)hipEventDestroy(used[i]); }
      if (cs) (void)hipStreamDestroy(cs);
    }
  } sd;
  unsigned long long *err; CHK(ws_get("g1codec.err", 8, (void **)&err));
  HIPCHK(hipMemsetAsync(err, 0xff, 8, g.stream));
  HIPCHK(hipStreamCreateWithFlags(&sd.cs, hipStreamNonBlocking));
  for (int i = 0; i < 2; i++) {
    HIPCHK(hipEventCreateWithFlags(&sd.copied[i], hipEventDisableTiming)); HIPCHK(hipEventCreateWithFlags(&sd.used[i], hipEventDisableTiming));
    HIPCHK(hipEventRecord(sd.copied[i], sd.cs)); HIPCHK(hipEventRecord(sd.used[i], g.stream));
  }
  uint64_t done = 0; int which = 0;
  while (done < sh.n) {
    const uint64_t len = std::min<uint64_t>(chunk_pts, sh.n - done);
    char *half = stage.at((uint64_t)which * chunk_pts * 32);
    HIPCHK(hipEventSynchronize(sd.copied[which]));
    if (fread(pinned[which], 1, len * 32, f) != len * 32) return fail(MI355_EBADARG, "srs_load_params_file: short read");
    HIPCHK(hipStreamWaitEvent(sd.cs, sd.used[which], 0));
    HIPCHK(hipMemcpyAsync(half, pinned[which], len * 32, hipMemcpyHostToDevice, sd.cs));
    HIPCHK(hipEventRecord(sd.copied[which], sd.cs));
    HIPCHK(hipStreamWaitEvent(g.stream, sd.copied[which], 0));
    CHK(launch_g1_decompress(half, sh.dev + done, len, sh.lo + done, err));
    HIPCHK(hipEventRecord(sd.used[which], g.stream));
    done += len; which ^= 1;
  }
  HIPCHK(hipMemcpyAsync(bad_out, err, 8, hipMemcpyDeviceToHost, g.stream));
  HIPCHK(hipStreamSynchronize(g.stream));
  return MI355_OK;
}
int mi355_srs_load_params_file(const char *path, uint32_t flags, uint32_t *k_out, uint64_t *g_handle_out, uint64_t *g_lagrange_handle_out, void *g2_out, void *s_g2_out) {
  return guarded([&]() -> int {
  AllGuard lk;
  CHK(need_init());
  if (!path || !k_out || !g_handle_out || !g_lagrange_handle_out) return fail(MI355_EBADARG, "srs_load_params_file: null pointer");
  FILE *f = fopen(path, "rb");
  if (!f) return fail(MI355_EBADARG, std::string("srs_load_params_file: cannot open ") + path);
  uint8_t hdr[4];
  int rc = MI355_OK; Srs sg, sl; void *pinned[2] = {nullptr, nullptr};
  do {
    if (fread(hdr, 1, 4, f) != 4) { rc = fail(MI355_EBADARG, "srs_load_params_file: empty file"); break; }
    const uint32_t k = (uint32_t)hdr[0] | ((uint32_t)hdr[1] << 8) | ((uint32_t)hdr[2] << 16) | ((uint32_t)hdr[3] << 24);
    if (k == 0 || k > 28) { rc = fail(MI355_EBADARG, "srs_load_params_file: k out of range (not a RawBytes params file)"); break; }
    const bool processed = (flags & 2u) != 0;
    const uint64_t n = 1ull << k, want = processed ? 4 + 2 * n * 32 + 128 : 4 + 2 * n * sizeof(g1_affine_t) + 256;
    if (fseek(f, 0, SEEK_END) != 0 || (uint64_t)ftell(f) != want) {
      rc = fail(MI355_EBADARG, processed ? "srs_load_params_file: file length does not match 4 + 2 * 2^k * 32 + 128 (not a Processed params file of this k)"
                                         : "srs_load_params_file: file length does not match 4 + 2 * 2^k * 64 + 256 (load_params rejects it too)");
      break;
    }
    fseek(f, 4, SEEK_SET);
    const size_t chunk = std::min<uint64_t>(64ull << 20, n * (processed ? 32 : sizeof(g1_affine_t)));
    sg.n = sl.n = n; sg.mem = std::make_shared<SrsMem>(); sl.mem = std::make_shared<SrsMem>();
    if (srs_alloc(*sg.mem, n) != MI355_OK || srs_alloc(*sl.mem, n) != MI355_OK) { (void)hipGetLastError(); rc = fail(MI355_EOOM, "srs_load_params_file: device allocation failed"); break; }
    bool okp = true;
    for (int i = 0; i < 2; i++) okp = okp && hipHostMalloc(&pinned[i], chunk, hipHostMallocPortable) == hipSuccess;
    if (!okp) { rc = fail(MI355_EOOM, "srs_load_params_file: pinned staging allocation failed"); break; }
    for (Srs *b : {&sg, &sl}) for (auto &sh : b->mem->sh) {
      if (rc != MI355_OK) break;
      if ((rc = bind_ctx(sh.slot)) != MI355_OK) break;
      if (!processed) { rc = stream_file_to_device(f, sh.dev, sh.n * sizeof(g1_affine_t), pinned, chunk); continue; }
      unsigned long long bad = ~0ull;
      rc = stream_processed_to_shard(f, sh, pinned, chunk / 32, &bad);
      if (rc == MI355_OK && bad != ~0ull)
        rc = fail(MI355_EBADARG, std::string("srs_load_params_file: ") + (b == &sg ? "g" : "g_lagrange") + "[" + std::to_string(bad) + "] is not the compressed form of a G1 point");
    }
    if (rc != MI355_OK) break;
    if (processed) {
      uint8_t tail[128]; uint8_t g2v[128], sg2v[128];
      if (fread(tail, 1, 128, f) != 128) { rc = fail(MI355_EBADARG, "srs_load_params_file: short read (g2 / s_g2)"); break; }
      if (!g2_decode_host(tail, g2v)) { rc = fail(MI355_EBADARG, "srs_load_params_file: g2 is not the compressed form of a point of the twist"); break; }
      if (!g2_decode_host(tail + 64, sg2v)) { rc = fail(MI355_EBADARG, "srs_load_params_file: s_g2 is not the compressed form of a point of the twist"); break; }
      if (g2_out) memcpy(g2_out, g2v, 128);
      if (s_g2_out) memcpy(s_g2_out, sg2v, 128);
      *k_out = k;
      *g_handle_out = srs_insert(sg);
      *g_lagrange_handle_out = srs_insert(sl);
      break;
    }
    uint8_t tail[256];
    if (fread(tail, 1, 256, f) != 256) { rc = fail(MI355_EBADARG, "srs_load_params_file: short read (g2 / s_g2)"); break; }
    if (g2_out) memcpy(g2_out, tail, 128);
    if (s_g2_out) memcpy(s_g2_out, tail + 128, 128);
    if (flags & 1u) {
      uint64_t nbad_total = 0;
      for (Srs *b : {&sg, &sl}) for (auto &sh : b->mem->sh) {
        if ((rc = bind_ctx(sh.slot)) != MI355_OK) break;
        uint32_t *bad = nullptr;
        if (ws_get("io.validate", 4, (void **)&bad) != MI355_OK) { rc = MI355_EHIP; break; }
        (void)hipMemsetAsync(bad, 0, 4, g.stream);
        hipLaunchKernelGGL(k_g1_validate, dim3(g.prop.multiProcessorCount * 8), dim3(256), 0, g.stream, sh.dev, sh.n, bad);
        uint32_t nbad = 0;
        if (hipMemcpyAsync(&nbad, bad, 4, hipMemcpyDeviceToHost, g.stream) != hipSuccess || hipStreamSynchronize(g.stream) != hipSuccess) { rc = fail(MI355_EHIP, "srs_load_params_file: validation failed to run"); break; }
        nbad_total += nbad;
      }
      if (rc != MI355_OK) break;
      if (nbad_total) { rc = fail(MI355_EBADARG, "srs_load_params_file: " + std::to_string(nbad_total) + " point(s) are not on the curve"); break; }
    }
    *k_out = k;
    *g_handle_out = srs_insert(sg);
    *g_lagrange_handle_out = srs_insert(sl);
  } while (false);
  fclose(f);
  for (int i = 0; i < 2; i++) if (pinned[i]) (void)hipHostFree(pinned[i]);
  const std::string keep = g_err;
  (void)bind_ctx(0);
  if (rc != MI355_OK) g_err = keep;
  return rc;
  });
}
int mi355_srs_precompute(uint64_t handle, uint64_t n_hint, int c) {
  return guarded([&]() -> int {
  AllGuard lk;
  CHK(need_init());
  Srs *sp; CHK(srs_find(handle, &sp, "srs_precompute"));
  SrsMem &mem = *sp->mem;
  if (n_hint == 0 || n_hint > sp->n) n_hint = sp->n;
  size_t live = 0; for (const auto &sh : mem.sh) if (sh.lo < sp->n) live++;
  const uint64_t per_shard = std::max<uint64_t>(1, n_hint / std::max<size_t>(1, live));
  const bool automatic = c == 0;
  if (automatic) {
    double best = 1e300;
    for (int cc = 4; cc <= (int)g_proc.msm_auto_max_c; cc++) { const double co = msm_cost(per_shard, cc, true); if (co < best) { best = co; c = cc; } }
  }
  if (c < 2 || c > MSM_MAX_C) return fail(MI355_EBADARG, "srs_precompute: window bits out of range");
  if (sp->tab) {
    if (sp->tab->c == c) return MI355_OK;
    if (automatic && msm_cost(per_shard, sp->tab->c, true) <= 1.10 * msm_cost(per_shard, c, true)) return MI355_OK;
  }
  const int W = (MSM_SCALAR_BITS + c - 1) / c;
  auto tab = std::make_shared<SrsTables>();
  tab->c = c; tab->w = W;
  tab->pre.assign(mem.sh.size(), nullptr); tab->stride.assign(mem.sh.size(), 0); tab->slot.assign(mem.sh.size(), 0);
  for (size_t i = 0; i < mem.sh.size(); i++) {
    const Shard &sh = mem.sh[i];
    tab->slot[i] = sh.slot;
    if (sh.lo >= sp->n) continue;
    const uint64_t cnt = std::min(sh.n, sp->n - sh.lo);
    CHK(bind_ctx(sh.slot));
    CHK(dev_malloc((void **)&tab->pre[i], (size_t)W * cnt * sizeof(g1_affine_t), "srs_precompute (window table)"));
    tab->stride[i] = cnt;
    hipLaunchKernelGGL(k_srs_precompute, dim3(ceil_div(cnt, 256)), dim3(256), 0, g.stream, sh.dev, tab->pre[i], cnt, (uint32_t)W, (uint32_t)c);
    HIPCHK(hipGetLastError());
  }
  for (const auto &sh : mem.sh) { CHK(bind_ctx(sh.slot)); HIPCHK(hipStreamSynchronize(g.stream)); }
  sp->tab = tab;
  return bind_ctx(0);
  });
}

struct Piece { int slot; const g1_affine_t *bases; PreTable pre; uint64_t a , cnt; };
static int srs_pieces(uint64_t handle, uint64_t off, uint64_t n, std::vector<Piece> &out) {
  Srs *sp; CHK(srs_find(handle, &sp, "msm"));
  if (off > sp->n || n > sp->n - off) return fail(MI355_EBADARG, "msm: base_offset + n exceeds the registered basis (best_multiexp panics on length mismatch)");
  const SrsMem &mem = *sp->mem;
  for (size_t i = 0; i < mem.sh.size(); i++) {
    const Shard &sh = mem.sh[i];
    const uint64_t lo = std::max(off, sh.lo), hi = std::min(off + n, sh.lo + sh.n);
    if (hi <= lo) continue;
    Piece p; p.slot = sh.slot; p.bases = sh.dev + (lo - sh.lo); p.a = lo - off; p.cnt = hi - lo;
    if (sp->tab && sp->tab->pre[i] && hi - sh.lo <= sp->tab->stride[i]) { p.pre.table = sp->tab->pre[i] + (lo - sh.lo); p.pre.row_stride = sp->tab->stride[i]; p.pre.c = sp->tab->c; p.pre.w = sp->tab->w; }
    out.push_back(p);
  }
  if (out.empty()) { Piece p; p.slot = 0; p.bases = nullptr; p.a = 0; p.cnt = 0; out.push_back(p); }
  return MI355_OK;
}

enum ScalarLoc { SCALARS_HOST = 0, SCALARS_DEV = 1 };
static int msm_multi(const std::vector<Piece> &pieces, const fe_t *const *polys, ScalarLoc loc, uint32_t M, void *out_host) {
  const int D = g_ndev;
  const MsmOpts opts = t_opts;
  std::vector<int> rcs(D, MI355_OK); std::vector<std::string> errs(D);
  std::vector<const Piece *> by_slot(D, nullptr);
  for (const auto &p : pieces) by_slot[p.slot] = &p;
  std::vector<int> owner(M, 0);
  if (loc == SCALARS_DEV) {
    bool seen[MAX_DEV] = {false};
    for (uint32_t m = 0; m < M; m++) { owner[m] = slot_of(polys[m]); seen[owner[m]] = true; }
    if (D > 1) for (int s = 0; s < D; s++) if (seen[s]) { CHK(bind_ctx(s)); HIPCHK(hipStreamSynchronize(g.stream)); }
  }
  auto work = [&](int slot) {
    t_opts = opts; t_opts.normalise = false;
    auto body = [&]() -> int {
      CHK(bind_ctx(slot));
      g1_jac_t *send; CHK(ws_get("xchg.send", (size_t)M * sizeof(g1_jac_t), (void **)&send));
      const Piece *p = by_slot[slot];
      if (!p || p->cnt == 0) { HIPCHK(hipMemsetAsync(send, 0, (size_t)M * sizeof(g1_jac_t), g.stream)); return MI355_OK; }
      std::vector<const fe_t *> ptrs(M);
      if (loc == SCALARS_HOST) {
        for (uint32_t m = 0; m < M; m++) ptrs[m] = polys[m] + p->a;
        return msm_host_single(p->bases, ptrs.data(), M, p->cnt, nullptr, &p->pre, send);
      }
      fe_t *sc = nullptr;
      for (uint32_t m = 0; m < M; m++) {
        const int o = owner[m];
        if (g_ctx[o].device == g.device) { ptrs[m] = polys[m] + p->a; continue; }
        if (!sc) CHK(ws_get("io.scalars", (size_t)M * p->cnt * sizeof(fe_t), (void **)&sc));
        ptrs[m] = sc + (size_t)m * p->cnt;
        HIPCHK(hipMemcpyPeerAsync(sc + (size_t)m * p->cnt, g.device, polys[m] + p->a, g_ctx[o].device, p->cnt * sizeof(fe_t), g.stream));
      }
      return msm_batch_impl(p->bases, ptrs.data(), M, p->cnt, nullptr, &p->pre, send);
    };
    rcs[slot] = guarded(body, "msm shard worker");
    if (rcs[slot] != MI355_OK) errs[slot] = g_err;
  };
  {
    struct Joiner { std::vector<std::thread> th; ~Joiner() { for (auto &t : th) if (t.joinable()) t.join(); } } workers;
    workers.th.reserve(D);
    for (int s = 1; s < D; s++) workers.th.emplace_back(work, s);
    work(0);
  }
  t_opts = opts;
  CHK(bind_ctx(0));
  for (int s = 0; s < D; s++) if (rcs[s] != MI355_OK) return fail(rcs[s], "device slot " + std::to_string(s) + ": " + errs[s]);
  const size_t part_bytes = (size_t)M * sizeof(g1_jac_t);
  std::vector<g1_jac_t *> send(D), recv(D);
  for (int s = 0; s < D; s++) { CHK(bind_ctx(s)); CHK(ws_get("xchg.send", part_bytes, (void **)&send[s])); CHK(ws_get("xchg.recv", part_bytes * D, (void **)&recv[s])); }
  if (g_ctx[0].comm) {
    int r = g_rccl.GroupStart(); if (r != 0) return rccl_fail("ncclGroupStart", r);
    for (int s = 0; s < D; s++) {
      CHK(bind_ctx(s));
      r = g_rccl.AllGather(send[s], recv[s], part_bytes,  1, g_ctx[s].comm, g_ctx[s].stream);
      if (r != 0) { (void)g_rccl.GroupEnd(); return rccl_fail("ncclAllGather", r); }
    }
    r = g_rccl.GroupEnd(); if (r != 0) return rccl_fail("ncclGroupEnd", r);
    g_last_exchange = "rccl_allgather";
  } else {
    for (int s = 0; s < D; s++) {
      CHK(bind_ctx(s)); HIPCHK(hipEventRecord(g.ev_xchg, g.stream));
      CHK(bind_ctx(0)); HIPCHK(hipStreamWaitEvent(g.stream, g_ctx[s].ev_xchg, 0));
      HIPCHK(hipMemcpyAsync((char *)recv[0] + part_bytes * s, send[s], part_bytes, hipMemcpyDeviceToDevice, g.stream));
    }
    g_last_exchange = "device_copy";
  }
  CHK(bind_ctx(0));
  g1_jac_t *res; CHK(ws_get("xchg.result", part_bytes, (void **)&res));
  hipLaunchKernelGGL(k_g1_sum_strided, dim3(M), dim3(64), 0, g.stream, (const g1_jac_t *)recv[0], (uint32_t)D, M, res, opts.normalise ? 1 : 0);
  HIPCHK(hipGetLastError());
  HIPCHK(hipMemcpyAsync(out_host, res, part_bytes, hipMemcpyDeviceToHost, g.stream));
  HIPCHK(hipStreamSynchronize(g.stream));
  for (int s = D - 1; s >= 0; s--) { CHK(bind_ctx(s)); if (s) HIPCHK(hipStreamSynchronize(g.stream)); resolve_spans(); }
  g_last_devices = D;
  return MI355_OK;
}
static bool single_device_call(const std::vector<Piece> &pieces) { return pieces.size() == 1 && pieces[0].slot == 0 && !g_proc.multi_force; }

static int msm_host_dispatch(uint64_t srs_handle, uint64_t base_offset, const void *const *scalars_host, uint32_t M, uint64_t n, void *out_g1_host) {
  std::vector<Piece> pieces; CHK(srs_pieces(srs_handle, base_offset, n, pieces));
  if (M == 0 || n == 0) { if (M) memset(out_g1_host, 0, (size_t)M * sizeof(g1_jac_t)); return MI355_OK; }
  if (!single_device_call(pieces)) return msm_multi(pieces, (const fe_t *const *)scalars_host, SCALARS_HOST, M, out_g1_host);
  const Piece &p = pieces[0];
  g_last_devices = 1; g_last_exchange = "none";
  const uint32_t group_max = (uint32_t)std::max<uint64_t>(1, (4ull << 30) / (n * sizeof(fe_t)));
  for (uint32_t m0 = 0; m0 < M; m0 += group_max) {
    const uint32_t mg = std::min(group_max, M - m0);
    CHK(msm_host_single(p.bases, (const fe_t *const *)scalars_host + m0, mg, n, (char *)out_g1_host + (size_t)m0 * sizeof(g1_jac_t), &p.pre));
  }
  return MI355_OK;
}
static int msm_dev_dispatch(uint64_t srs_handle, uint64_t base_offset, const void *const *scalars_dev, uint32_t M, uint64_t n, void *out_g1_host) {
  std::vector<Piece> pieces; CHK(srs_pieces(srs_handle, base_offset, n, pieces));
  if (M == 0 || n == 0) { if (M) memset(out_g1_host, 0, (size_t)M * sizeof(g1_jac_t)); return MI355_OK; }
  if (!single_device_call(pieces)) return msm_multi(pieces, (const fe_t *const *)scalars_dev, SCALARS_DEV, M, out_g1_host);
  g_last_devices = 1; g_last_exchange = "none";
  std::vector<const fe_t *> ptrs(M);
  fe_t *stage = nullptr; size_t staged = 0;
  for (uint32_t m = 0; m < M; m++) {
    const int o = slot_of(scalars_dev[m], true);
    ptrs[m] = (const fe_t *)scalars_dev[m];
    if (g_ndev > 1 && o != 0) {
      CHK(bind_ctx(o)); HIPCHK(hipStreamSynchronize(g.stream));
      if (!g_peer_ok[0][o]) {
        CHK(bind_ctx(0));
        if (!stage) CHK(ws_get("io.scalars", (size_t)M * n * sizeof(fe_t), (void **)&stage));
        HIPCHK(hipMemcpyPeerAsync(stage + staged, g.device, scalars_dev[m], g_ctx[o].device, n * sizeof(fe_t), g.stream));
        ptrs[m] = stage + staged; staged += n;
      }
    }
  }
  CHK(bind_ctx(0));
  return msm_batch_impl(pieces[0].bases, ptrs.data(), M, n, out_g1_host, &pieces[0].pre);
}

int mi355_msm_g1_dev(uint64_t srs_handle, uint64_t base_offset, const void *scalars_dev, uint64_t n, void *out_g1_host) {
  return guarded([&]() -> int {
  MsmGuard lk;
  CHK(need_init());
  if (!out_g1_host || (n && !scalars_dev)) return fail(MI355_EBADARG, "msm: null pointer");
  return msm_dev_dispatch(srs_handle, base_offset, &scalars_dev, 1, n, out_g1_host);
  });
}
int mi355_msm_g1_dev_async(uint64_t srs_handle, uint64_t base_offset, const void *scalars_dev, uint64_t n, void *out_g1_dev) {
  return guarded([&]() -> int {
  MsmGuard lk;
  CHK(need_init());
  if (!out_g1_dev || (n && !scalars_dev)) return fail(MI355_EBADARG, "msm: null pointer");
  std::vector<Piece> pieces; CHK(srs_pieces(srs_handle, base_offset, n, pieces));
  if (pieces.size() != 1 || pieces[0].slot != 0) return fail(MI355_EBADARG, "msm_g1_dev_async: the range must lie on the primary device (one process per GPU drives its own shard)");
  const fe_t *sc = (const fe_t *)scalars_dev;
  (void)slot_of(scalars_dev, true); (void)slot_of(out_g1_dev, true);
  return msm_batch_impl(pieces[0].bases, &sc, 1, n, nullptr, &pieces[0].pre, out_g1_dev);
  });
}
int mi355_g1_sum_dev(const void *pts_dev, uint64_t n, void *out_g1_host) {
  return guarded([&]() -> int {
  const int slot = slot_of(pts_dev);
  DevGuard lk(slot);
  CHK(need_init(slot));
  if (!out_g1_host || (n && !pts_dev) || n > (1u << 20)) return fail(MI355_EBADARG, "g1_sum: bad argument");
  g1_jac_t *dev; CHK(ws_get("io.g1sum", sizeof(g1_jac_t), (void **)&dev));
  hipLaunchKernelGGL(k_g1_sum, dim3(1), dim3(64), 0, g.stream, (const g1_jac_t *)pts_dev, (uint32_t)n, dev);
  HIPCHK(hipGetLastError());
  HIPCHK(hipMemcpyAsync(out_g1_host, dev, sizeof(g1_jac_t), hipMemcpyDeviceToHost, g.stream));
  HIPCHK(hipStreamSynchronize(g.stream));
  return MI355_OK;
  });
}
int mi355_msm_g1_host(uint64_t srs_handle, uint64_t base_offset, const void *scalars_host, uint64_t n, void *out_g1_host) {
  return guarded([&]() -> int {
  MsmGuard lk;
  CHK(need_init());
  if (!out_g1_host || (n && !scalars_host)) return fail(MI355_EBADARG, "msm: null pointer");
  return msm_host_dispatch(srs_handle, base_offset, &scalars_host, 1, n, out_g1_host);
  });
}
int mi355_msm_g1_batch_dev(uint64_t srs_handle, uint64_t base_offset, const void *const *scalars_dev, uint32_t batch, uint64_t n, void *out_g1_host) {
  return guarded([&]() -> int {
  MsmGuard lk;
  CHK(need_init());
  if (!out_g1_host || (batch && !scalars_dev)) return fail(MI355_EBADARG, "msm_batch: null pointer");
  for (uint32_t m = 0; m < batch; m++) if (n && !scalars_dev[m]) return fail(MI355_EBADARG, "msm_batch: null polynomial pointer");
  return msm_dev_dispatch(srs_handle, base_offset, scalars_dev, batch, n, out_g1_host);
  });
}
int mi355_msm_g1_batch_host(uint64_t srs_handle, uint64_t base_offset, const void *const *scalars_host, uint32_t batch, uint64_t n, void *out_g1_host) {
  return guarded([&]() -> int {
  MsmGuard lk;
  CHK(need_init());
  if (!out_g1_host || (batch && !scalars_host)) return fail(MI355_EBADARG, "msm_batch: null pointer");
  for (uint32_t m = 0; m < batch; m++) if (n && !scalars_host[m]) return fail(MI355_EBADARG, "msm_batch: null polynomial pointer");
  return msm_host_dispatch(srs_handle, base_offset, scalars_host, batch, n, out_g1_host);
  });
}
int mi355_msm_set_pipeline(uint32_t chunks, uint32_t min_log_n) {
  return guarded([&]() -> int {
  AllGuard lk;
  if (chunks > 16 || min_log_n > 31) return fail(MI355_EBADARG, "msm_set_pipeline: chunks <= 16, min_log_n <= 31");
  for (int s = 0; s < std::max(1, g_ndev); s++) { g_ctx[s].msm_chunks = chunks ? chunks : 1; g_ctx[s].msm_chunk_min_log = chunks ? min_log_n : 23; }
  return MI355_OK;
  });
}
int mi355_msm_g1_adhoc_host(const void *bases_host, const void *scalars_host, uint64_t n, void *out_g1_host) {
  return guarded([&]() -> int {
  MsmGuard lk;
  CHK(need_init());
  if (!out_g1_host || (n && (!scalars_host || !bases_host))) return fail(MI355_EBADARG, "msm: null pointer");
  fe_t *sc = nullptr; g1_affine_t *bs = nullptr;
  if (n) {
    CHK(ws_get("io.scalars", n * sizeof(fe_t), (void **)&sc)); CHK(ws_get("io.bases", n * sizeof(g1_affine_t), (void **)&bs));
    HIPCHK(hipMemcpyAsync(sc, scalars_host, n * sizeof(fe_t), hipMemcpyHostToDevice, g.stream));
    HIPCHK(hipMemcpyAsync(bs, bases_host, n * sizeof(g1_affine_t), hipMemcpyHostToDevice, g.stream));
  }
  g_last_devices = 1; g_last_exchange = "none";
  const fe_t *poly = sc;
  return msm_batch_impl(bs, &poly, 1, n, out_g1_host, nullptr);
  });
}
int mi355_msm_g1_segmented_host(const void *bases_affine_host, const void *scalars_host, const uint64_t *offsets_host, uint32_t segments, void *out_g1affine_host) {
  return guarded([&]() -> int {
  if (segments > (1u << 20)) return fail(MI355_EBADARG, "msm_segmented: more than 2^20 segments");
  uint64_t total = 0;
  if (segments) {
    if (!offsets_host || !out_g1affine_host) return fail(MI355_EBADARG, "msm_segmented: null pointer");
    if (offsets_host[0] != 0) return fail(MI355_EBADARG, "msm_segmented: offsets[0] must be 0");
    for (uint32_t s = 0; s < segments; s++) if (offsets_host[s + 1] < offsets_host[s]) return fail(MI355_EBADARG, "msm_segmented: offsets decrease at segment " + std::to_string(s));
    total = offsets_host[segments];
    if (total > (1ull << 24)) return fail(MI355_EBADARG, "msm_segmented: more than 2^24 terms (this entry point is for many SHORT segments)");
    if (total && (!bases_affine_host || !scalars_host)) return fail(MI355_EBADARG, "msm_segmented: null pointer");
  }
  MsmGuard lk;
  CHK(need_init());
  if (segments == 0) return MI355_OK;
  if (total == 0) { memset(out_g1affine_host, 0, (size_t)segments * sizeof(g1_affine_t)); return MI355_OK; }
  CallTrace tr("msm_g1_segmented", total, 96.0);
  hipStream_t s = g.stream;
  fe_t *sc; g1_affine_t *bs, *out_dev; uint64_t *off;
  CHK(ws_get("io.scalars", total * sizeof(fe_t), (void **)&sc)); CHK(ws_get("io.bases", total * sizeof(g1_affine_t), (void **)&bs));
  CHK(ws_get("msmseg.offsets", ((size_t)segments + 1) * 8, (void **)&off)); CHK(ws_get("msmseg.out", (size_t)segments * sizeof(g1_affine_t), (void **)&out_dev));
  HIPCHK(hipMemcpyAsync(sc, scalars_host, total * sizeof(fe_t), hipMemcpyHostToDevice, s));
  HIPCHK(hipMemcpyAsync(bs, bases_affine_host, total * sizeof(g1_affine_t), hipMemcpyHostToDevice, s));
  HIPCHK(hipMemcpyAsync(off, offsets_host, ((size_t)segments + 1) * 8, hipMemcpyHostToDevice, s));
  {
    Scope sp("msm_segmented", s);
    hipLaunchKernelGGL(k_msm_g1_segmented, dim3(segments), dim3(SEGMSM_LANES), 0, s, (const g1_affine_t *)bs, (const fe_t *)sc, (const uint64_t *)off, out_dev);
    HIPCHK(hipGetLastError());
  }
  HIPCHK(hipMemcpyAsync(out_g1affine_host, out_dev, (size_t)segments * sizeof(g1_affine_t), hipMemcpyDeviceToHost, s));
  HIPCHK(hipStreamSynchronize(s));
  resolve_spans();
  { char buf[48]; snprintf(buf, sizeof buf, " segments=%u", segments); tr.done(buf); }
  return MI355_OK;
  });
}
int mi355_g1_sum_host(const void *pts_host, uint64_t n, void *out_g1_host) {
  return guarded([&]() -> int {
  DevGuard lk(0);
  CHK(need_init());
  if (!out_g1_host || (n && !pts_host) || n > (1u << 20)) return fail(MI355_EBADARG, "g1_sum: bad argument");
  g1_jac_t *dev; CHK(ws_get("io.g1sum", (n + 1) * sizeof(g1_jac_t), (void **)&dev));
  if (n) HIPCHK(hipMemcpyAsync(dev + 1, pts_host, n * sizeof(g1_jac_t), hipMemcpyHostToDevice, g.stream));
  hipLaunchKernelGGL(k_g1_sum, dim3(1), dim3(64), 0, g.stream, dev + 1, (uint32_t)n, dev);
  HIPCHK(hipGetLastError());
  HIPCHK(hipMemcpyAsync(out_g1_host, dev, sizeof(g1_jac_t), hipMemcpyDeviceToHost, g.stream));
  HIPCHK(hipStreamSynchronize(g.stream));
  return MI355_OK;
  });
}
int mi355_msm_set_window_bits(int c) {
  return guarded([&]() -> int {
  if (c == -1) { t_opts.force_c = 0; t_opts.no_tables = true; return MI355_OK; }
  if (c != 0 && (c < 2 || c > MSM_MAX_C)) return fail(MI355_EBADARG, "window bits must be 0 (auto), -1 (auto, no window tables) or in [2, 24]");
  t_opts.force_c = c; t_opts.no_tables = false; return MI355_OK;
  });
}
int mi355_msm_set_normalise(int on) { t_opts.normalise = on != 0; return MI355_OK; }
int mi355_msm_last_plan(int *c_out, int *windows_out, uint64_t *entries_out) {
  return guarded([&]() -> int {
  DevGuard lk(0);
  const Ctx &p = g_ctx[0];
  if (c_out) *c_out = p.last_c; if (windows_out) *windows_out = p.last_w; if (entries_out) *entries_out = p.last_entries; return MI355_OK;
  });
}
int mi355_msm_last_run(int *devices_out, const char **exchange_out, int *shared_tables_out, int *host_slices_out) {
  return guarded([&]() -> int {
  DevGuard lk(0);
  if (devices_out) *devices_out = g_last_devices; if (exchange_out) *exchange_out = g_last_exchange;
  if (shared_tables_out) *shared_tables_out = g_ctx[0].last_shared ? 1 : 0; if (host_slices_out) *host_slices_out = g_ctx[0].last_host_slices;
  return MI355_OK;
  });
}

int mi355_msm_g2_adhoc_host(const void *bases_g2affine_host, const void *scalars_host, uint64_t n, void *out_g2affine_host) {
  return guarded([&]() -> int {
  MsmGuard lk;
  CHK(need_init());
  if (!out_g2affine_host || (n && (!scalars_host || !bases_g2affine_host))) return fail(MI355_EBADARG, "msm_g2: null pointer");
  if (n >= (1ull << 31)) return fail(MI355_EBADARG, "msm_g2: n must be < 2^31");
  fe_t *sc = nullptr; g2_affine_t *bs = nullptr;
  if (n) {
    CHK(ws_get("io.scalars", n * sizeof(fe_t), (void **)&sc)); CHK(ws_get("io.g2_bases", n * sizeof(g2_affine_t), (void **)&bs));
    HIPCHK(hipMemcpyAsync(sc, scalars_host, n * sizeof(fe_t), hipMemcpyHostToDevice, g.stream));
    HIPCHK(hipMemcpyAsync(bs, bases_g2affine_host, n * sizeof(g2_affine_t), hipMemcpyHostToDevice, g.stream));
  }
  const fe_t *p = sc;
  return msm_g2_run(bs, &p, 1, n, out_g2affine_host);
  });
}
static int g2_dev_operand(const void *p) {
  if (slot_of(p, true) != 0) return fail(MI355_EBADARG, "msm_g2: bases and scalars must live on the primary device (G2 MSMs run on one device)");
  return MI355_OK;
}
int mi355_msm_g2_dev(const void *bases_g2affine_dev, const void *scalars_dev, uint64_t n, void *out_g2affine_host) {
  return guarded([&]() -> int {
  MsmGuard lk;
  CHK(need_init());
  if (!out_g2affine_host || (n && (!scalars_dev || !bases_g2affine_dev))) return fail(MI355_EBADARG, "msm_g2: null pointer");
  if (n) { CHK(g2_dev_operand(bases_g2affine_dev)); CHK(g2_dev_operand(scalars_dev)); }
  CHK(bind_ctx(0));
  const fe_t *p = (const fe_t *)scalars_dev;
  return msm_g2_run((const g2_affine_t *)bases_g2affine_dev, &p, 1, n, out_g2affine_host);
  });
}
int mi355_msm_g2_batch_dev(const void *bases_g2affine_dev, const void *const *scalars_dev, uint32_t batch, uint64_t n, void *out_g2affine_host) {
  return guarded([&]() -> int {
  MsmGuard lk;
  CHK(need_init());
  if (!out_g2affine_host || (batch && !scalars_dev) || (batch && n && !bases_g2affine_dev)) return fail(MI355_EBADARG, "msm_g2_batch: null pointer");
  for (uint32_t m = 0; m < batch; m++) if (n && !scalars_dev[m]) return fail(MI355_EBADARG, "msm_g2_batch: null polynomial pointer");
  if (batch && n) { CHK(g2_dev_operand(bases_g2affine_dev)); for (uint32_t m = 0; m < batch; m++) CHK(g2_dev_operand(scalars_dev[m])); }
  CHK(bind_ctx(0));
  if (batch == 0) return MI355_OK;
  return msm_g2_run((const g2_affine_t *)bases_g2affine_dev, (const fe_t *const *)scalars_dev, batch, n, out_g2affine_host);
  });
}

static int ensure_fixed_base_table() {
  if (g.fixed_base_table) return MI355_OK;
  CHK(dev_malloc((void **)&g.fixed_base_table, 32 * 256 * sizeof(g1_affine_t), "fixed-base table"));
  hipLaunchKernelGGL(k_fixed_base_table, dim3(1), dim3(256), 0, g.stream, g.fixed_base_table);
  HIPCHK(hipGetLastError());
  return MI355_OK;
}
int mi355_g1_fixed_base_mul_dev(void *points_dev, const void *scalars_dev, uint64_t n) {
  return guarded([&]() -> int {
  int slot; CHK(common_slot({points_dev, scalars_dev}, &slot, "fixed_base_mul"));
  DevGuard lk(slot);
  CHK(need_init(slot));
  if (!points_dev || !scalars_dev) return fail(MI355_EBADARG, "fixed_base_mul: null pointer");
  CHK(ensure_fixed_base_table());
  hipLaunchKernelGGL(k_fixed_base_mul, dim3(ceil_div(n, 256)), dim3(256), 0, g.stream, g.fixed_base_table, (const fe_t *)scalars_dev, (g1_affine_t *)points_dev, n);
  HIPCHK(hipGetLastError());
  return MI355_OK;
  });
}
int mi355_srs_setup_dev(void *g_dev, void *g_lagrange_dev, uint32_t k, const void *tau, const void *omega) {
  return guarded([&]() -> int {
  int slot; CHK(common_slot({g_dev, g_lagrange_dev}, &slot, "srs_setup"));
  DevGuard lk(slot);
  CHK(need_init(slot));
  if (!g_dev || !g_lagrange_dev || !tau || !omega || k > 28) return fail(MI355_EBADARG, "srs_setup: bad argument");
  CHK(ensure_fixed_base_table());
  const uint64_t n = 1ull << k;
  fe_t *sc; CHK(ws_get("srs.scalars", 2 * n * sizeof(fe_t), (void **)&sc));
  fe_t t, w; memcpy(&t, tau, 32); memcpy(&w, omega, 32);
  fe_t nn = Fr::zero(); nn.l[0] = (uint32_t)n; nn.l[1] = (uint32_t)(n >> 32);
  const fe_t tn1_over_n = Fr::mul(Fr::sub(Fr::pow_u64(t, n), Fr::one()), Fr::inv(Fr::from_canonical(nn)));
  hipLaunchKernelGGL(k_srs_scalars, dim3(ceil_div(n, 256)), dim3(256), 0, g.stream, sc, sc + n, t, w, tn1_over_n, n);
  hipLaunchKernelGGL(k_fixed_base_mul, dim3(ceil_div(n, 256)), dim3(256), 0, g.stream, g.fixed_base_table, sc, (g1_affine_t *)g_dev, n);
  hipLaunchKernelGGL(k_fixed_base_mul, dim3(ceil_div(n, 256)), dim3(256), 0, g.stream, g.fixed_base_table, sc + n, (g1_affine_t *)g_lagrange_dev, n);
  HIPCHK(hipGetLastError());
  HIPCHK(hipStreamSynchronize(g.stream));
  return MI355_OK;
  });
}

}
```

### scroll-prover_amd/csrc/msm.hpp

```cpp
#pragma once
#include "fp_asm.hpp"
#include "g1_29.hpp"
#include "frscan.hpp"

namespace zk {

#if defined(__HIPCC__)

struct MsmPlan {
  uint32_t n;
  uint32_t c;
  uint32_t windows;
  uint32_t nb;
  uint32_t seg;
  uint32_t batch;
};

__device__ __forceinline__ g1_affine_t load_affine(const g1_affine_t *p) {
  g1_affine_t r; r.x = g_load(&p->x); r.y = g_load(&p->y); return r;
}
__device__ __forceinline__ g1_affine_t load_affine_nt(const g1_affine_t *p) {
  const uint32_t *q = reinterpret_cast<const uint32_t *>(p); g1_affine_t r;
#pragma unroll
  for (int i = 0; i < 8; i++) { r.x.l[i] = __builtin_nontemporal_load(q + i); r.y.l[i] = __builtin_nontemporal_load(q + 8 + i); }
  return r;
}
__device__ __forceinline__ g1_xyzz_t load_xyzz(const g1_xyzz_t *p) {
  g1_xyzz_t r; r.x = g_load(&p->x); r.y = g_load(&p->y); r.zz = g_load(&p->zz); r.zzz = g_load(&p->zzz); return r;
}
__device__ __forceinline__ void store_xyzz(g1_xyzz_t *p, const g1_xyzz_t &v) {
  g_store(&p->x, v.x); g_store(&p->y, v.y); g_store(&p->zz, v.zz); g_store(&p->zzz, v.zzz);
}

__device__ __forceinline__ void store_xyzz29(g1_xyzz29_t *p, const g1_xyzz29_t &v) {
  const uint32_t *w = reinterpret_cast<const uint32_t *>(&v); uint4 *q = reinterpret_cast<uint4 *>(p);
#pragma unroll
  for (int i = 0; i < 9; i++) q[i] = make_uint4(w[4 * i], w[4 * i + 1], w[4 * i + 2], w[4 * i + 3]);
}
__device__ __forceinline__ g1_xyzz29_t load_xyzz29(const g1_xyzz29_t *p) {
  g1_xyzz29_t v; uint32_t *w = reinterpret_cast<uint32_t *>(&v); const uint4 *q = reinterpret_cast<const uint4 *>(p);
#pragma unroll
  for (int i = 0; i < 9; i++) { const uint4 a = q[i]; w[4 * i] = a.x; w[4 * i + 1] = a.y; w[4 * i + 2] = a.z; w[4 * i + 3] = a.w; }
  return v;
}

__device__ __forceinline__ g1_xyzz29_t shfl_down_xyzz29(const g1_xyzz29_t &v, uint32_t o) {
  g1_xyzz29_t r; const uint32_t *s = reinterpret_cast<const uint32_t *>(&v); uint32_t *d = reinterpret_cast<uint32_t *>(&r);
#pragma unroll
  for (int i = 0; i < 36; i++) d[i] = __shfl_down(s[i], o);
  return r;
}
__device__ __forceinline__ g1_xyzz29_t shfl_xor_xyzz29(const g1_xyzz29_t &v, uint32_t o) {
  g1_xyzz29_t r; const uint32_t *s = reinterpret_cast<const uint32_t *>(&v); uint32_t *d = reinterpret_cast<uint32_t *>(&r);
#pragma unroll
  for (int i = 0; i < 36; i++) d[i] = __shfl_xor(s[i], o);
  return r;
}

template <int J> __device__ __forceinline__ fe29_t quad_bcast(const fe29_t &v) {
  fe29_t r;
#pragma unroll
  for (int i = 0; i < 9; i++) {
    int x = __builtin_amdgcn_mov_dpp((int)v.l[i], J * 0x55, 0xf, 0xf, true);
    asm volatile("" : "+v"(x));
    r.l[i] = (uint32_t)x;
  }
  return r;
}
__device__ __forceinline__ fe29_t quad_sel(uint32_t q, const fe29_t a0, const fe29_t a1, const fe29_t a2, const fe29_t a3) {
  fe29_t r;
#pragma unroll
  for (int i = 0; i < 9; i++) { const uint32_t x0 = a0.l[i], x1 = a1.l[i], x2 = a2.l[i], x3 = a3.l[i]; const uint32_t lo = q & 1u ? x1 : x0, hi = q & 1u ? x3 : x2; r.l[i] = q & 2u ? hi : lo; }
  return r;
}
__device__ __forceinline__ g1_xyzz29_t g1_xyzz29_dbl_q4(const g1_xyzz29_t &a) {
  if (g1_xyzz29_is_identity(a)) return a;
  const uint32_t q = threadIdx.x & 3u;
  const fe29_t xt = Fq29::reduce_small(Fq29::normalise(a.x));
  const fe29_t yc = Fq29::carry(a.y);
  const fe29_t U = Fq29::dbl(yc);
  fe29_t m = Fq29::mul_c(quad_sel(q, U, xt, U, xt), quad_sel(q, U, xt, U, xt));
  const fe29_t V = quad_bcast<0>(m), xx = quad_bcast<1>(m);
  const fe29_t M = Fq29::carry(Fq29::add(Fq29::dbl(xx), xx));
  m = Fq29::mul_c(quad_sel(q, U, xt, M, V), quad_sel(q, V, V, M, a.zz));
  const fe29_t W = quad_bcast<0>(m), S = quad_bcast<1>(m), MM = quad_bcast<2>(m), ZZ3 = quad_bcast<3>(m);
  g1_xyzz29_t r;
  r.x = Fq29::sub8(MM, Fq29::dbl(S));
  const fe29_t t = Fq29::sub16(S, r.x);
  m = Fq29::mul_c(quad_sel(q, M, W, W, W), quad_sel(q, t, yc, a.zzz, a.zzz));
  r.y = Fq29::sub4(quad_bcast<0>(m), quad_bcast<1>(m));
  r.zz = ZZ3; r.zzz = quad_bcast<2>(m);
  return r;
}
__device__ __forceinline__ void g1_xyzz29_add_q4(g1_xyzz29_t &acc, const g1_xyzz29_t &o) {
  if (g1_xyzz29_is_identity(o)) return;
  if (g1_xyzz29_is_identity(acc)) { acc = o; return; }
  const uint32_t q = threadIdx.x & 3u;
  fe29_t m = Fq29::mul_c(quad_sel(q, acc.x, acc.y, o.x, o.y), quad_sel(q, o.zz, o.zzz, acc.zz, acc.zzz));
  const fe29_t U1 = quad_bcast<0>(m), S1 = quad_bcast<1>(m), U2 = quad_bcast<2>(m), S2 = quad_bcast<3>(m);
  const fe29_t Pd = Fq29::sub4(U2, U1), Rd = Fq29::sub4(S2, S1);
  m = Fq29::mul_c(quad_sel(q, Pd, Rd, acc.zz, acc.zzz), quad_sel(q, Pd, Rd, o.zz, o.zzz));
  const fe29_t PP = quad_bcast<0>(m), RR = quad_bcast<1>(m), ZZ12 = quad_bcast<2>(m), ZZZ12 = quad_bcast<3>(m);
  const fe29_t one = Fq29::one();
  m = Fq29::mul_c(quad_sel(q, Pd, U1, ZZ12, Rd), quad_sel(q, PP, PP, PP, one));
  const fe29_t PPP = quad_bcast<0>(m), Q = quad_bcast<1>(m), ZZ3 = quad_bcast<2>(m), Rone = quad_bcast<3>(m);
  if (Fq29::is_zero_tight(ZZ3)) {
    if (Fq29::is_zero_tight(Rone)) acc = g1_xyzz29_dbl_q4(acc);
    else acc = g1_xyzz29_identity();
    return;
  }
  const fe29_t X3 = Fq29::sub4_8(RR, PPP, Fq29::dbl(Q));
  const fe29_t t = Fq29::sub16(Q, X3);
  m = Fq29::mul_c(quad_sel(q, Rd, S1, ZZZ12, ZZZ12), quad_sel(q, t, PPP, PPP, PPP));
  acc.x = X3; acc.y = Fq29::sub4(quad_bcast<0>(m), quad_bcast<1>(m));
  acc.zz = ZZ3; acc.zzz = quad_bcast<2>(m);
}
template <int Q> __device__ __forceinline__ void g1_vadd(g1_xyzz29_t &acc, const g1_xyzz29_t &o) { if (Q == 4) g1_xyzz29_add_q4(acc, o); else g1_xyzz29_add(acc, o); }
template <int Q> __device__ __forceinline__ g1_xyzz29_t g1_vdbl(const g1_xyzz29_t &a) { return Q == 4 ? g1_xyzz29_dbl_q4(a) : g1_xyzz29_dbl(a); }

__device__ __forceinline__ void msm_emit_result(const g1_xyzz_t &acc, g1_jac_t *out, int normalise) {
  if (normalise) { *out = g1_xyzz_to_jac_normalised(acc); return; }
  g1_jac_t r;
  if (g1_xyzz_is_identity(acc)) { r.x = Fq::zero(); r.y = Fq::zero(); r.z = Fq::zero(); }
  else { r.x = FqPs::mul(acc.x, FqPs::sqr(acc.zz)); r.y = FqPs::mul(acc.y, FqPs::sqr(acc.zzz)); r.z = acc.zzz; }
  *out = r;
}

struct G1Ops {
  using rec_t = g1_xyzz29_t; using out_t = g1_jac_t;
  static constexpr bool QUAD = true;
  static constexpr const char *ROLE = "msm.";
  static __device__ __forceinline__ rec_t identity() { return g1_xyzz29_identity(); }
  static __device__ __forceinline__ rec_t load(const rec_t *p) { return load_xyzz29(p); }
  static __device__ __forceinline__ void store(rec_t *p, const rec_t &v) { store_xyzz29(p, v); }
  template <int Q> static __device__ __forceinline__ void add(rec_t &acc, const rec_t &o) { g1_vadd<Q>(acc, o); }
  template <int Q> static __device__ __forceinline__ rec_t dbl(const rec_t &a) { return g1_vdbl<Q>(a); }
  static __device__ __forceinline__ rec_t shfl_down(const rec_t &v, uint32_t o) { return shfl_down_xyzz29(v, o); }
  static __device__ __forceinline__ void emit(const rec_t &acc, out_t *out, int normalise) { msm_emit_result(g1_xyzz29_to_sat(acc), out, normalise); }
};

struct PolyPtrs { const fe_t *p[8]; };
template <bool FOLD>
__global__ void __launch_bounds__(256) k_msm_digits(PolyPtrs inl, const fe_t *const *__restrict__ polys, uint32_t *__restrict__ enc, MsmPlan P,
                                                     uint32_t *__restrict__ coarse_hist, uint32_t fb, uint32_t cb_bits, uint32_t shared) {
  extern __shared__ uint32_t hist_lds[];
  const uint32_t CB = 1u << cb_bits, per_poly = (shared ? 1u : P.windows) * CB, regions = P.batch * per_poly;
  for (uint32_t b = threadIdx.x; b < regions; b += blockDim.x) hist_lds[b] = 0;
  __syncthreads();
  const uint32_t stride = gridDim.x * blockDim.x, m = blockIdx.y;
  const fe_t *__restrict__ poly = polys ? polys[m] : inl.p[m];
  const uint32_t half = 1u << (P.c - 1), mask = (1u << P.c) - 1;
  for (uint32_t i = blockIdx.x * blockDim.x + threadIdx.x; i < P.n; i += stride) {
    const fe_t k = Fr::redc(g_load(&poly[i]));
    fe_t t; { uint32_t borrow = 0;
#pragma unroll
      for (int q = 0; q < 8; q++) { const uint64_t d = (uint64_t)FrP::mod(q) - k.l[q] - borrow; t.l[q] = (uint32_t)d; borrow = (uint32_t)(d >> 63); } }
    bool flip = false;
#pragma unroll
    for (int q = 7; q >= 0; q--) { if (t.l[q] != k.l[q]) { flip = FOLD && t.l[q] < k.l[q]; break; } }
    const uint32_t sign_flip = flip ? 0x80000000u : 0u;
    uint32_t l0 = flip ? t.l[0] : k.l[0], l1 = flip ? t.l[1] : k.l[1], l2 = flip ? t.l[2] : k.l[2], l3 = flip ? t.l[3] : k.l[3];
    uint32_t l4 = flip ? t.l[4] : k.l[4], l5 = flip ? t.l[5] : k.l[5], l6 = flip ? t.l[6] : k.l[6], l7 = flip ? t.l[7] : k.l[7];
    uint32_t carry = 0;
    for (uint32_t w = 0; w < P.windows; w++) {
      const uint32_t raw = (l0 & mask) + carry;
      l0 = __funnelshift_r(l0, l1, P.c); l1 = __funnelshift_r(l1, l2, P.c); l2 = __funnelshift_r(l2, l3, P.c); l3 = __funnelshift_r(l3, l4, P.c);
      l4 = __funnelshift_r(l4, l5, P.c); l5 = __funnelshift_r(l5, l6, P.c); l6 = __funnelshift_r(l6, l7, P.c); l7 >>= P.c;
      uint32_t e;
      if (raw > half) { e = (1u << P.c) - raw; if (e) e |= 0x80000000u; carry = 1; } else { e = raw; carry = 0; }
      if (e) e ^= sign_flip;
      enc[((uint64_t)m * P.windows + w) * P.n + i] = e;
      if (e) atomicAdd(&hist_lds[m * per_poly + (shared ? 0 : w * CB) + (((e & 0x7fffffffu) - 1) >> fb)], 1u);
    }
  }
  __syncthreads();
  for (uint32_t b = threadIdx.x; b < regions; b += blockDim.x) if (hist_lds[b]) atomicAdd(&coarse_hist[b], hist_lds[b]);
}

constexpr uint32_t SCAN_BLOCK = 1024, SCAN_ITEMS = 4;
__device__ __forceinline__ uint32_t block_exclusive_scan(uint32_t v, uint32_t *lds, uint32_t &total) {
  const uint32_t lane = threadIdx.x & 63, wave = threadIdx.x >> 6;
  uint32_t x = v;
  for (uint32_t o = 1; o < 64; o <<= 1) { uint32_t y = __shfl_up(x, o); if (lane >= o) x += y; }
  if (lane == 63) lds[wave] = x;
  __syncthreads();
  if (wave == 0) { uint32_t s = lane < (blockDim.x >> 6) ? lds[lane] : 0; for (uint32_t o = 1; o < 16; o <<= 1) { uint32_t y = __shfl_up(s, o); if (lane >= o) s += y; } if (lane < 16) lds[16 + lane] = s; }
  __syncthreads();
  const uint32_t wave_off = wave ? lds[16 + wave - 1] : 0;
  total = lds[16 + (blockDim.x >> 6) - 1];
  __syncthreads();
  return wave_off + x - v;
}
__global__ void __launch_bounds__(SCAN_BLOCK) k_scan_partial(const uint32_t *__restrict__ in, uint32_t *__restrict__ block_sums, uint32_t n) {
  __shared__ uint32_t lds[32];
  const uint32_t base = blockIdx.x * SCAN_BLOCK * SCAN_ITEMS + threadIdx.x * SCAN_ITEMS;
  uint32_t s = 0;
  for (uint32_t k = 0; k < SCAN_ITEMS; k++) if (base + k < n) s += in[base + k];
  uint32_t total; block_exclusive_scan(s, lds, total);
  if (threadIdx.x == 0) block_sums[blockIdx.x] = total;
}
__global__ void __launch_bounds__(SCAN_BLOCK) k_scan_block_sums(uint32_t *block_sums, uint32_t nblocks) {
  __shared__ uint32_t lds[32];
  __shared__ uint32_t running;
  if (threadIdx.x == 0) running = 0;
  __syncthreads();
  for (uint32_t base = 0; base < nblocks; base += SCAN_BLOCK) {
    const uint32_t i = base + threadIdx.x;
    const uint32_t v = i < nblocks ? block_sums[i] : 0;
    uint32_t total; const uint32_t ex = block_exclusive_scan(v, lds, total);
    const uint32_t r = running;
    if (i < nblocks) block_sums[i] = r + ex;
    __syncthreads();
    if (threadIdx.x == 0) running = r + total;
    __syncthreads();
  }
}
__global__ void __launch_bounds__(SCAN_BLOCK) k_scan_final(const uint32_t *__restrict__ in, const uint32_t *__restrict__ block_sums, uint32_t *__restrict__ out_a, uint32_t *__restrict__ out_b, uint32_t n) {
  __shared__ uint32_t lds[32];
  const uint32_t base = blockIdx.x * SCAN_BLOCK * SCAN_ITEMS + threadIdx.x * SCAN_ITEMS;
  uint32_t v[SCAN_ITEMS], s = 0;
  for (uint32_t k = 0; k < SCAN_ITEMS; k++) { v[k] = base + k < n ? in[base + k] : 0; s += v[k]; }
  uint32_t total; uint32_t ex = block_exclusive_scan(s, lds, total) + block_sums[blockIdx.x];
  for (uint32_t k = 0; k < SCAN_ITEMS; k++) if (base + k < n) { out_a[base + k] = ex; out_b[base + k] = ex; ex += v[k]; }
}

constexpr uint32_t SORT_MAX_BINS = 4096;
constexpr uint32_t SORT_SPLIT_TMAX = 128;
struct SortPlan { uint32_t n, windows , wpp , nb, fb, cb_bits, t1, t2, regions, shared, nshift ; };

__device__ __forceinline__ uint32_t tile_bin_offsets(const uint32_t *h, uint32_t *lstart, uint32_t (&gb)[4], uint32_t nbins, uint32_t *global_cursor, uint32_t *scratch32) {
  const uint32_t bpt = (nbins + 1023) >> 10, b0 = threadIdx.x * bpt;
  uint32_t local[4], sum = 0;
  for (uint32_t k = 0; k < 4; k++) { local[k] = (k < bpt && b0 + k < nbins) ? h[b0 + k] : 0; sum += local[k]; }
  uint32_t total; uint32_t ex = block_exclusive_scan(sum, scratch32, total);
  for (uint32_t k = 0; k < 4; k++) { gb[k] = 0; if (k < bpt && b0 + k < nbins) { lstart[b0 + k] = ex; if (local[k]) gb[k] = atomicAdd(&global_cursor[b0 + k], local[k]); ex += local[k]; } }
  return total;
}
__device__ __forceinline__ void tile_bin_publish(uint32_t *gbase, const uint32_t *lstart, const uint32_t (&gb)[4], uint32_t nbins) {
  const uint32_t bpt = (nbins + 1023) >> 10, b0 = threadIdx.x * bpt;
  for (uint32_t k = 0; k < 4; k++) if (k < bpt && b0 + k < nbins) gbase[b0 + k] = gb[k] - lstart[b0 + k];
}
template <int EPT> __global__ void __launch_bounds__(1024) k_sort_l1_scatter_split(const uint32_t *__restrict__ enc, uint32_t *__restrict__ coarse_cursor, uint32_t *__restrict__ pairs_lo,
                                                                                    uint16_t *__restrict__ pairs_hi, SortPlan S) {
  extern __shared__ uint32_t sm[];
  const uint32_t CB = 1u << S.cb_bits, CBp = (CB + 1) & ~1u, fmask = (1u << S.fb) - 1;
  const uint32_t spare = 16u - S.fb, rmask = (1u << spare) - 1, tcount = (CB + rmask) >> spare;
  uint32_t *h = sm, *lstart = sm + CBp, *gbase = sm + 2 * CBp, *scratch32 = sm + 3 * CBp, *T = sm + 3 * CBp + 32;
  uint32_t *stage_lo = T + SORT_SPLIT_TMAX;
  uint16_t *stage_hi = reinterpret_cast<uint16_t *>(stage_lo + 1024 * EPT);
  const uint32_t tiles1 = (S.n + S.t1 - 1) / S.t1;
  const uint32_t w = blockIdx.x / tiles1, j = blockIdx.x - w * tiles1;
  for (uint32_t b = threadIdx.x; b < CB; b += 1024) h[b] = 0;
  __syncthreads();
  const uint32_t i0 = j * S.t1, i1 = min(S.n, i0 + S.t1);
  const uint32_t *plane = enc + (uint64_t)w * S.n;
  uint32_t e[EPT], rank[EPT];
#pragma unroll
  for (int k = 0; k < EPT; k++) {
    const uint32_t i = i0 + k * 1024 + threadIdx.x;
    e[k] = i < i1 ? plane[i] : 0;
  }
  asm volatile("s_waitcnt vmcnt(0)" ::: "memory");
#pragma unroll
  for (int k = 0; k < EPT; k++) if (e[k]) rank[k] = atomicAdd(&h[((e[k] & 0x7fffffffu) - 1) >> S.fb], 1u);
  __syncthreads();
  const uint32_t m_poly = w / S.wpp, w_in = w - m_poly * S.wpp;
  uint32_t gb[4];
  const uint32_t total = tile_bin_offsets(h, lstart, gb, CB, coarse_cursor + (S.shared ? m_poly * CB : w * CB), scratch32);
  const uint32_t idx_base = S.shared ? w_in << S.nshift : 0;
  __syncthreads();
  for (uint32_t k = threadIdx.x; k < tcount; k += 1024) T[k] = lstart[k << spare];
#pragma unroll
  for (int k = 0; k < EPT; k++) if (e[k]) {
    const uint32_t bucket = (e[k] & 0x7fffffffu) - 1, i = i0 + k * 1024 + threadIdx.x, bin = bucket >> S.fb, pos = lstart[bin] + rank[k];
    stage_lo[pos] = (idx_base + i) | (e[k] & 0x80000000u);
    stage_hi[pos] = (uint16_t)((bucket & fmask) | ((bin & rmask) << S.fb));
  }
  tile_bin_publish(gbase, lstart, gb, CB);
  __syncthreads();
  uint32_t k = 0;
  for (uint32_t sidx = threadIdx.x; sidx < total; sidx += 1024) {
    const uint32_t key = stage_hi[sidx];
    while (k + 1 < tcount && T[k + 1] <= sidx) k++;
    const uint32_t bin = (k << spare) | (key >> S.fb), pos = gbase[bin] + sidx;
    pairs_lo[pos] = stage_lo[sidx]; pairs_hi[pos] = (uint16_t)(key & fmask);
  }
}
__global__ void __launch_bounds__(SCAN_BLOCK) k_sort_tile_prefix(const uint32_t *__restrict__ coarse_off, uint32_t *__restrict__ tile_start, SortPlan S) {
  __shared__ uint32_t lds[32];
  __shared__ uint32_t running;
  if (threadIdx.x == 0) running = 0;
  __syncthreads();
  for (uint32_t base = 0; base < S.regions; base += SCAN_BLOCK) {
    const uint32_t r = base + threadIdx.x;
    const uint32_t v = r < S.regions ? (coarse_off[r + 1] - coarse_off[r] + S.t2 - 1) / S.t2 : 0;
    uint32_t total; const uint32_t ex = block_exclusive_scan(v, lds, total);
    const uint32_t run = running;
    if (r < S.regions) tile_start[r] = run + ex;
    __syncthreads();
    if (threadIdx.x == 0) running = run + total;
    __syncthreads();
  }
  if (threadIdx.x == 0) tile_start[S.regions] = running;
}
__device__ __forceinline__ bool sort_l2_tile(const uint32_t *__restrict__ coarse_off, const uint32_t *__restrict__ tile_start, const SortPlan &S, uint32_t &region, uint32_t &s, uint32_t &e) {
  const uint32_t total = tile_start[S.regions], per_xcd = (total + 7) >> 3, q = blockIdx.x >> 3;
  const uint32_t tile = (blockIdx.x & 7) * per_xcd + q;
  if (q >= per_xcd || tile >= total) return false;
  uint32_t lo = 0, hi = S.regions;
  while (hi - lo > 1) { const uint32_t mid = (lo + hi) >> 1; if (tile_start[mid] <= tile) lo = mid; else hi = mid; }
  region = lo;
  s = coarse_off[lo] + (tile - tile_start[lo]) * S.t2;
  e = min(coarse_off[lo + 1], s + S.t2);
  return true;
}
__global__ void __launch_bounds__(256) k_sort_l2_hist_split(const uint16_t *__restrict__ pairs_hi, const uint32_t *__restrict__ coarse_off, const uint32_t *__restrict__ tile_start,
                                                            uint32_t *__restrict__ hist, SortPlan S) {
  __shared__ uint32_t h[SORT_MAX_BINS];
  uint32_t region, s, e;
  if (!sort_l2_tile(coarse_off, tile_start, S, region, s, e)) return;
  const uint32_t FB = 1u << S.fb;
  for (uint32_t b = threadIdx.x; b < FB; b += blockDim.x) h[b] = 0;
  __syncthreads();
  const uint32_t a0 = min(e, (s + 7u) & ~7u), a1 = a0 + ((e - a0) & ~7u);
  for (uint32_t p = s + threadIdx.x; p < a0; p += blockDim.x) atomicAdd(&h[pairs_hi[p]], 1u);
  for (uint32_t q = a0 + 8u * threadIdx.x; q < a1; q += 8u * blockDim.x) {
    const uint4 v = *reinterpret_cast<const uint4 *>(pairs_hi + q);
    atomicAdd(&h[v.x & 0xffffu], 1u); atomicAdd(&h[v.x >> 16], 1u); atomicAdd(&h[v.y & 0xffffu], 1u); atomicAdd(&h[v.y >> 16], 1u);
    atomicAdd(&h[v.z & 0xffffu], 1u); atomicAdd(&h[v.z >> 16], 1u); atomicAdd(&h[v.w & 0xffffu], 1u); atomicAdd(&h[v.w >> 16], 1u);
  }
  for (uint32_t p = a1 + threadIdx.x; p < e; p += blockDim.x) atomicAdd(&h[pairs_hi[p]], 1u);
  __syncthreads();
  for (uint32_t b = threadIdx.x; b < FB; b += blockDim.x) if (h[b]) atomicAdd(&hist[(region << S.fb) + b], h[b]);
}
template <int EPT> __global__ void __launch_bounds__(1024) k_sort_l2_scatter_split(const uint32_t *__restrict__ pairs_lo, const uint16_t *__restrict__ pairs_hi, const uint32_t *__restrict__ coarse_off,
                                                                                    const uint32_t *__restrict__ tile_start, uint32_t *__restrict__ cursor, uint32_t *__restrict__ sorted, SortPlan S) {
  extern __shared__ uint32_t sm[];
  const uint32_t FB = 1u << S.fb;
  uint32_t *h = sm, *lstart = sm + FB, *gbase = sm + 2 * FB, *scratch32 = sm + 3 * FB, *stage = sm + 3 * FB + 32;
  uint32_t region, s, e;
  if (!sort_l2_tile(coarse_off, tile_start, S, region, s, e)) return;
  for (uint32_t b = threadIdx.x; b < FB; b += 1024) h[b] = 0;
  __syncthreads();
  uint32_t idx[EPT], fine[EPT], rank[EPT];
#pragma unroll
  for (int k = 0; k < EPT; k++) {
    const uint32_t p = s + k * 1024 + threadIdx.x;
    fine[k] = 0xffffffffu;
    if (p < e) { idx[k] = pairs_lo[p]; fine[k] = pairs_hi[p]; }
  }
  asm volatile("s_waitcnt vmcnt(0)" ::: "memory");
#pragma unroll
  for (int k = 0; k < EPT; k++) if (fine[k] != 0xffffffffu) rank[k] = atomicAdd(&h[fine[k]], 1u);
  __syncthreads();
  uint32_t gb[4];
  const uint32_t total = tile_bin_offsets(h, lstart, gb, FB, cursor + (region << S.fb), scratch32);
  __syncthreads();
  uint16_t *stage_bin = reinterpret_cast<uint16_t *>(stage + 1024 * EPT);
#pragma unroll
  for (int k = 0; k < EPT; k++) if (fine[k] != 0xffffffffu) { const uint32_t pos = lstart[fine[k]] + rank[k]; stage[pos] = idx[k]; stage_bin[pos] = (uint16_t)fine[k]; }
  tile_bin_publish(gbase, lstart, gb, FB);
  __syncthreads();
  for (uint32_t sidx = threadIdx.x; sidx < total; sidx += 1024) {
    const uint32_t b = stage_bin[sidx];
    sorted[gbase[b] + sidx] = stage[sidx];
  }
}

__device__ __forceinline__ uint32_t msm_seg_eff(uint32_t total, uint32_t threads, uint32_t seg_arg) {
  const uint32_t seg_max = seg_arg & 0x1fffu, seg_min = (seg_arg >> 13) & 0x1fffu, fill_pct = (seg_arg >> 26) * 2;
  const uint64_t target = ((uint64_t)threads * (fill_pct > 100u ? 100u : fill_pct) + 99) / 100;
  uint32_t sg = (uint32_t)(((uint64_t)total + target - 1) / (target ? target : 1));
  sg = sg < seg_min ? seg_min : sg;
  return sg > seg_max ? seg_max : sg;
}
template <class G, class B> __device__ __forceinline__ void msm_segment_walk(const B &bases, const uint32_t *__restrict__ sorted, const uint32_t *__restrict__ offsets, uint32_t nbuckets,
                                                                              typename G::rec_t *__restrict__ bucket_sums, typename G::rec_t *__restrict__ part, int32_t *__restrict__ part_id, uint32_t seg_arg,
                                                                              uint32_t t, uint32_t threads) {
  const uint32_t total = offsets[nbuckets];
  const uint32_t seg = msm_seg_eff(total, threads, seg_arg);
  const uint64_t start64 = (uint64_t)t * seg;
  if (start64 >= total) { part_id[2 * t] = -1; part_id[2 * t + 1] = -1; return; }
  const uint32_t start = (uint32_t)start64, end = (uint32_t)min((uint64_t)total, start64 + seg);
  uint32_t lo = 0, hi = nbuckets;
  while (hi - lo > 1) { const uint32_t mid = (lo + hi) >> 1; if (offsets[mid] <= start) lo = mid; else hi = mid; }
  uint32_t b = lo, b_start = offsets[b], b_end = offsets[b + 1];
  int32_t id_first = -1, id_last = -1;
  typename G::rec_t acc = G::identity();
  uint32_t ent = sorted[start];
  uint32_t ent_next = start + 1 < end ? sorted[start + 1] : 0;
  typename B::base_t p = bases.load(ent);
  for (uint32_t pos = start; pos < end; pos++) {
    typename B::base_t p_next = p;
    if (pos + 1 < end) { ent_next = sorted[pos + 1]; p_next = bases.load(ent_next); }
    if (pos >= b_end) {
      if (b_start >= start) G::store(&bucket_sums[b], acc);
      else { G::store(&part[2 * (uint64_t)t], acc); id_first = (int32_t)b; }
      acc = G::identity();
      b++; b_start = b_end; b_end = offsets[b + 1];
      if (pos >= b_end) {
        uint32_t l2 = b, h2 = nbuckets;
        while (h2 - l2 > 1) { const uint32_t mid = (l2 + h2) >> 1; if (offsets[mid] <= pos) l2 = mid; else h2 = mid; }
        b = l2; b_start = offsets[b]; b_end = offsets[b + 1];
      }
    }
    bases.madd(acc, p, (ent >> 31) != 0);
    ent = ent_next; p = p_next;
  }
  if (b_start >= start && b_end <= end) G::store(&bucket_sums[b], acc);
  else if (b_start < start) { G::store(&part[2 * (uint64_t)t], acc); id_first = (int32_t)b; }
  else { G::store(&part[2 * (uint64_t)t + 1], acc); id_last = (int32_t)b; }
  part_id[2 * t] = id_first; part_id[2 * t + 1] = id_last;
}
struct G1Bases {
  using base_t = g1_affine_t;
  const g1_affine_t *__restrict__ bases; uint32_t nshift; uint64_t row_stride;
  __device__ __forceinline__ const g1_affine_t *base_of(uint32_t e) const {
    const uint32_t gi = e & 0x7fffffffu;
    if (row_stride == 0) return &bases[gi];
    const uint32_t w = gi >> nshift;
    return &bases[(uint64_t)w * row_stride + (gi & ((1u << nshift) - 1))];
  }
  __device__ __forceinline__ g1_affine_t load(uint32_t e) const { return load_affine(base_of(e)); }
  __device__ __forceinline__ void madd(g1_xyzz29_t &acc, const g1_affine_t &p, bool neg) const { g1_xyzz29_madd(acc, p, neg); }
};
struct G1AccOps : G1Ops {
  static __device__ __forceinline__ void store(rec_t *p, rec_t v) { g1_xyzz29_negx_to_plain(v); store_xyzz29(p, v); }
};
__global__ void __launch_bounds__(256) k_msm_accumulate(const g1_affine_t *__restrict__ bases, const uint32_t *__restrict__ sorted, const uint32_t *__restrict__ offsets,
                                                        uint32_t nbuckets, g1_xyzz29_t *__restrict__ bucket_sums, g1_xyzz29_t *__restrict__ part, int32_t *__restrict__ part_id, uint32_t seg_arg,
                                                        uint32_t nshift, uint64_t row_stride) {
  msm_segment_walk<G1AccOps>(G1Bases{bases, nshift, row_stride}, sorted, offsets, nbuckets, bucket_sums, part, part_id, seg_arg, blockIdx.x * blockDim.x + threadIdx.x, gridDim.x * blockDim.x);
}

constexpr uint32_t FIXUP_SERIAL_MAX = 32, FIXUP_HUGE_MIN = 2048, FIXUP_SLICES = 64;
template <int Q = 1> __device__ __forceinline__ void fixup_take29(g1_xyzz29_t &acc, const g1_xyzz29_t *__restrict__ part, const int32_t *__restrict__ part_id, uint32_t t, uint32_t b) {
  if (part_id[2 * t] == (int32_t)b) g1_vadd<Q>(acc, load_xyzz29(&part[2 * (uint64_t)t]));
  else if (part_id[2 * t + 1] == (int32_t)b) g1_vadd<Q>(acc, load_xyzz29(&part[2 * (uint64_t)t + 1]));
}
template <uint32_t FIXUP_LANES, int Q = 1> __global__ void __launch_bounds__(256) k_msm_fixup(const uint32_t *__restrict__ offsets, uint32_t nbuckets, g1_xyzz29_t *__restrict__ bucket_sums,
                                                   const g1_xyzz29_t *__restrict__ part, const int32_t *__restrict__ part_id, uint32_t seg_arg, uint32_t acc_threads,
                                                   uint32_t *__restrict__ big_list, uint32_t *__restrict__ big_count, uint32_t big_cap,
                                                   uint32_t *__restrict__ huge_list, uint32_t *__restrict__ huge_count, uint32_t huge_cap, uint32_t serial_max, uint32_t huge_min) {
  const uint32_t gid = (blockIdx.x * blockDim.x + threadIdx.x) / Q, b = gid / FIXUP_LANES, sub = gid % FIXUP_LANES;
  const bool lead = (threadIdx.x & (Q - 1)) == 0;
  const uint32_t seg = msm_seg_eff(offsets[nbuckets], acc_threads, seg_arg);
  g1_xyzz29_t acc = g1_xyzz29_identity();
  bool mine = false;
  if (b < nbuckets) {
    const uint32_t s = offsets[b], e = offsets[b + 1];
    if (e != s) {
      const uint32_t t0 = s / seg, t1 = (e - 1) / seg;
      if (t0 != t1) {
        if (t1 - t0 > serial_max) {
          if (sub == 0 && lead) {
            if (huge_cap && t1 - t0 >= huge_min) {
              const uint32_t idx = atomicAdd(huge_count, 1u);
              if (idx < huge_cap) { huge_list[3 * idx] = b; huge_list[3 * idx + 1] = t0; huge_list[3 * idx + 2] = t1; }
            } else {
              const uint32_t idx = atomicAdd(big_count, 1u);
              if (idx < big_cap) { big_list[3 * idx] = b; big_list[3 * idx + 1] = t0; big_list[3 * idx + 2] = t1; }
            }
          }
        } else {
          mine = true;
          for (uint32_t t = t0 + sub; t <= t1; t += FIXUP_LANES) fixup_take29<Q>(acc, part, part_id, t, b);
        }
      }
    }
  }
  if (FIXUP_LANES > 1) { const g1_xyzz29_t other = shfl_xor_xyzz29(acc, 1 * Q); g1_vadd<Q>(acc, other); }
  if (FIXUP_LANES > 2) { const g1_xyzz29_t other = shfl_xor_xyzz29(acc, 2 * Q); g1_vadd<Q>(acc, other); }
  static_assert(FIXUP_LANES == 1 || FIXUP_LANES == 2 || FIXUP_LANES == 4, "two shuffle steps");
  if (mine && sub == 0 && lead) store_xyzz29(&bucket_sums[b], acc);
}
__global__ void __launch_bounds__(256) k_msm_fixup_big(g1_xyzz29_t *__restrict__ bucket_sums, const g1_xyzz29_t *__restrict__ part, const int32_t *__restrict__ part_id,
                                                       const uint32_t *__restrict__ big_list, const uint32_t *__restrict__ big_count) {
  __shared__ g1_xyzz29_t lds29[4];
  if (blockIdx.x >= *big_count) return;
  const uint32_t b = big_list[3 * blockIdx.x], t0 = big_list[3 * blockIdx.x + 1], t1 = big_list[3 * blockIdx.x + 2];
  g1_xyzz29_t acc = g1_xyzz29_identity();
  for (uint32_t t = t0 + threadIdx.x; t <= t1; t += blockDim.x) fixup_take29(acc, part, part_id, t, b);
  for (uint32_t o = 32; o >= 1; o >>= 1) { const g1_xyzz29_t other = shfl_down_xyzz29(acc, o); g1_xyzz29_add(acc, other); }
  if ((threadIdx.x & 63) == 0) lds29[threadIdx.x >> 6] = acc;
  __syncthreads();
  if (threadIdx.x == 0) { for (uint32_t k = 1; k < (blockDim.x >> 6); k++) g1_xyzz29_add(acc, lds29[k]); store_xyzz29(&bucket_sums[b], acc); }
}
__device__ __forceinline__ uint32_t fixup_huge_slices(uint32_t span) { const uint32_t s = span >> 11; return s < 1u ? 1u : (s > FIXUP_SLICES ? FIXUP_SLICES : s); }
__global__ void __launch_bounds__(256) k_msm_fixup_huge(const g1_xyzz29_t *__restrict__ part, const int32_t *__restrict__ part_id, const uint32_t *__restrict__ huge_list,
                                                        const uint32_t *__restrict__ huge_count, g1_xyzz29_t *__restrict__ huge_part, uint32_t huge_cap) {
  __shared__ g1_xyzz29_t lds29[4];
  const uint32_t count = min(*huge_count, huge_cap);
  if (count == 0) return;
  const uint32_t sl = blockIdx.x / count, idx = blockIdx.x - sl * count;
  if (sl >= FIXUP_SLICES) return;
  const uint32_t b = huge_list[3 * idx], t0 = huge_list[3 * idx + 1], t1 = huge_list[3 * idx + 2], span = t1 - t0 + 1;
  const uint32_t nsl = fixup_huge_slices(span);
  if (sl >= nsl) return;
  const uint32_t lo = t0 + (uint32_t)((uint64_t)span * sl / nsl), hi = t0 + (uint32_t)((uint64_t)span * (sl + 1) / nsl);
  g1_xyzz29_t acc = g1_xyzz29_identity();
  for (uint32_t t = lo + threadIdx.x; t < hi; t += blockDim.x) fixup_take29(acc, part, part_id, t, b);
  for (uint32_t o = 32; o >= 1; o >>= 1) { const g1_xyzz29_t other = shfl_down_xyzz29(acc, o); g1_xyzz29_add(acc, other); }
  if ((threadIdx.x & 63) == 0) lds29[threadIdx.x >> 6] = acc;
  __syncthreads();
  if (threadIdx.x == 0) { for (uint32_t k = 1; k < (blockDim.x >> 6); k++) g1_xyzz29_add(acc, lds29[k]); store_xyzz29(&huge_part[(uint64_t)idx * FIXUP_SLICES + sl], acc); }
}
__global__ void __launch_bounds__(64) k_msm_fixup_huge_fold(g1_xyzz29_t *__restrict__ bucket_sums, const uint32_t *__restrict__ huge_list, const uint32_t *__restrict__ huge_count,
                                                            const g1_xyzz29_t *__restrict__ huge_part) {
  const uint32_t idx = blockIdx.x;
  if (idx >= *huge_count) return;
  const uint32_t nsl = fixup_huge_slices(huge_list[3 * idx + 2] - huge_list[3 * idx + 1] + 1);
  g1_xyzz29_t acc = threadIdx.x < nsl ? load_xyzz29(&huge_part[(uint64_t)idx * FIXUP_SLICES + threadIdx.x]) : g1_xyzz29_identity();
  for (uint32_t o = FIXUP_SLICES / 2; o >= 1; o >>= 1) { const g1_xyzz29_t other = shfl_down_xyzz29(acc, o); g1_xyzz29_add(acc, other); }
  if (threadIdx.x == 0) store_xyzz29(&bucket_sums[huge_list[3 * idx]], acc);
}

template <class G> __global__ void __launch_bounds__(256) k_msm_segfix(const int32_t *__restrict__ ids, const typename G::rec_t *__restrict__ recs, uint32_t n, typename G::rec_t *__restrict__ bucket_sums,
                                                    int32_t *__restrict__ ids_out, typename G::rec_t *__restrict__ recs_out, int last_level) {
  using rec_t = typename G::rec_t;
  const uint32_t j = blockIdx.x * blockDim.x + threadIdx.x, lane = threadIdx.x & 63, wave = j >> 6;
  if (wave >= ((n + 63) >> 6)) return;
  const int32_t key0 = j < n ? ids[j] : -1;
  rec_t val = key0 >= 0 ? G::load(&recs[j]) : G::identity();
  int32_t key = key0;
  for (uint32_t o = 1; o < 64; o <<= 1) { const int32_t kk = __shfl_up(key, o); if (lane >= o && key < 0) key = kk; }
  for (uint32_t o = 1; o < 64; o <<= 1) {
    const int32_t k2 = __shfl_down(key, o);
    const bool take = lane + o < 64 && key >= 0 && k2 == key;
    if (__ballot(take) == 0) continue;
    const rec_t other = G::shfl_down(val, o);
    if (take) G::template add<1>(val, other);
  }
  const int32_t kprev = __shfl_up(key, 1);
  const bool head = key >= 0 && (lane == 0 || kprev != key);
  const uint64_t valid = __ballot(key >= 0);
  const uint32_t first_lane = valid ? (uint32_t)__ffsll((unsigned long long)valid) - 1 : 64u;
  const int32_t key_last = __shfl(key, 63), key_first = __shfl(key, first_lane < 64u ? (int)first_lane : 0);
  const bool is_first = head && lane == first_lane, is_last = head && key == key_last;
  if (last_level) { if (head) G::store(&bucket_sums[key], val); return; }
  if (head && !is_first && !is_last) G::store(&bucket_sums[key], val);
  if (is_first) { ids_out[2 * wave] = key; G::store(&recs_out[2 * (uint64_t)wave], val); }
  if (is_last && !is_first) { ids_out[2 * wave + 1] = key; G::store(&recs_out[2 * (uint64_t)wave + 1], val); }
  if (lane == 0) {
    if (first_lane == 64u) { ids_out[2 * wave] = -1; ids_out[2 * wave + 1] = -1; }
    else if (key_first == key_last) ids_out[2 * wave + 1] = -1;
  }
}

__global__ void __launch_bounds__(256) k_msm_bucket_fold(g1_xyzz29_t *__restrict__ buckets, uint32_t nbuckets, uint32_t sets) {
  const uint32_t b = blockIdx.x * blockDim.x + threadIdx.x;
  if (b >= nbuckets) return;
  g1_xyzz29_t acc = load_xyzz29(&buckets[b]);
  for (uint32_t k = 1; k < sets; k++) g1_xyzz29_add(acc, load_xyzz29(&buckets[(uint64_t)k * nbuckets + b]));
  store_xyzz29(&buckets[b], acc);
}

template <class G, int Q> __global__ void __launch_bounds__(128) k_msm_bucket_reduce(const typename G::rec_t *__restrict__ bucket_sums, typename G::rec_t *__restrict__ chunk_out, uint32_t nb, uint32_t sets, uint32_t chunk) {
  using rec_t = typename G::rec_t;
  const uint32_t chunks_per_set = nb / chunk;
  const uint32_t gi = (blockIdx.x * blockDim.x + threadIdx.x) / Q;
  if (gi >= chunks_per_set * sets) return;
  const uint32_t w = gi / chunks_per_set, j = gi - w * chunks_per_set;
  const rec_t *B = bucket_sums + (uint64_t)w * nb + (uint64_t)j * chunk;
  rec_t run = G::identity(), T = G::identity();
  for (uint32_t i = chunk; i-- > 0;) { G::template add<Q>(run, G::load(&B[i])); G::template add<Q>(T, run); }
  if (j != 0) {
    const uint32_t k = j * chunk;
    rec_t kS = G::identity();
    for (int bit = 31 - __clz(k); bit >= 0; bit--) { kS = G::template dbl<Q>(kS); if ((k >> bit) & 1) G::template add<Q>(kS, run); }
    G::template add<Q>(T, kS);
  }
  if ((threadIdx.x & (Q - 1)) == 0) G::store(&chunk_out[gi], T);
}
constexpr uint32_t TREE_PER_THREAD = 4;
template <class G, int Q> __global__ void __launch_bounds__(256) k_msm_tree_sum(const typename G::rec_t *__restrict__ in, uint32_t in_per_set, typename G::rec_t *__restrict__ out, uint32_t out_per_set) {
  using rec_t = typename G::rec_t;
  __shared__ rec_t lds[4];
  constexpr uint32_t VT = 256 / Q;
  const uint32_t w = blockIdx.y, first = blockIdx.x * VT * TREE_PER_THREAD, vt = threadIdx.x / Q;
  const rec_t *src = in + (uint64_t)w * in_per_set;
  rec_t acc = G::identity();
  for (uint32_t k = 0; k < TREE_PER_THREAD; k++) { const uint32_t i = first + k * VT + vt; if (i < in_per_set) G::template add<Q>(acc, G::load(&src[i])); }
  for (uint32_t o = 32 / Q; o >= 1; o >>= 1) { const rec_t other = G::shfl_down(acc, o * Q); G::template add<Q>(acc, other); }
  if ((threadIdx.x & 63) == 0) lds[threadIdx.x >> 6] = acc;
  __syncthreads();
  if (threadIdx.x < Q) { for (uint32_t k = 1; k < 4; k++) G::template add<Q>(acc, lds[k]); if (threadIdx.x == 0) G::store(&out[(uint64_t)w * out_per_set + blockIdx.x], acc); }
}
template <class G, int Q> __global__ void __launch_bounds__(64) k_msm_final(const typename G::rec_t *__restrict__ window_sums, uint32_t windows, uint32_t c, typename G::out_t *__restrict__ out, int normalise) {
  if (threadIdx.x >= Q) return;
  window_sums += (uint64_t)blockIdx.x * windows; out += blockIdx.x;
  typename G::rec_t acc = G::identity();
  for (uint32_t w = windows; w-- > 0;) {
    for (uint32_t k = 0; k < c; k++) acc = G::template dbl<Q>(acc);
    G::template add<Q>(acc, G::load(&window_sums[w]));
  }
  if (threadIdx.x == 0) G::emit(acc, out, normalise);
}
__global__ void k_g1_sum(const g1_jac_t *__restrict__ pts, uint32_t n, g1_jac_t *__restrict__ out) {
  if (threadIdx.x != 0 || blockIdx.x != 0) return;
  g1_xyzz_t acc = g1_xyzz_identity();
  for (uint32_t i = 0; i < n; i++) { g1_jac_t p = pts[i]; g1_xyzz_add<FqPs>(acc, g1_jac_to_xyzz(p)); }
  *out = g1_xyzz_to_jac_normalised(acc);
}

__global__ void k_g1_sum_strided(const g1_jac_t *__restrict__ pts, uint32_t count, uint32_t stride, g1_jac_t *__restrict__ out, int normalise) {
  if (threadIdx.x != 0) return;
  g1_xyzz_t acc = g1_xyzz_identity();
  for (uint32_t k = 0; k < count; k++) { g1_jac_t p = pts[(size_t)k * stride + blockIdx.x]; g1_xyzz_add<FqPs>(acc, g1_jac_to_xyzz(p)); }
  if (normalise) { out[blockIdx.x] = g1_xyzz_to_jac_normalised(acc); return; }
  g1_jac_t r;
  if (g1_xyzz_is_identity(acc)) { r.x = Fq::zero(); r.y = Fq::zero(); r.z = Fq::zero(); }
  else { r.x = FqPs::mul(acc.x, FqPs::sqr(acc.zz)); r.y = FqPs::mul(acc.y, FqPs::sqr(acc.zzz)); r.z = acc.zzz; }
  out[blockIdx.x] = r;
}

__global__ void __launch_bounds__(256) k_g1_validate(const g1_affine_t *__restrict__ pts, uint64_t n, uint32_t *__restrict__ bad) {
  uint32_t local = 0;
  for (uint64_t i = (uint64_t)blockIdx.x * blockDim.x + threadIdx.x; i < n; i += (uint64_t)gridDim.x * blockDim.x) {
    const g1_affine_t p = load_affine(&pts[i]);
    if (g1_affine_is_identity(p)) continue;
    bool ok = true;
    for (int c = 0; c < 2 && ok; c++) {
      const fe_t &v = c ? p.y : p.x; bool lt = false;
      for (int k = 7; k >= 0; k--) { if (v.l[k] != FqP::mod(k)) { lt = v.l[k] < FqP::mod(k); break; } }
      ok = lt;
    }
    if (ok) {
      fe_t three = Fq::zero(); three.l[0] = 3; three = Fq::from_canonical(three);
      ok = Fq::eq(FqPs::sqr(p.y), Fq::add(FqPs::mul(FqPs::sqr(p.x), p.x), three));
    }
    if (!ok) local++;
  }
  if (local) atomicAdd(bad, local);
}

__global__ void __launch_bounds__(FRSCAN_THREADS) k_srs_precompute(const g1_affine_t *__restrict__ base, g1_affine_t *__restrict__ table, uint64_t n, uint32_t W, uint32_t c) {
  __shared__ uint32_t buf[2 * FRSCAN_THREADS * 9];
  __shared__ uint32_t inv_total[8];
  const uint64_t i = (uint64_t)blockIdx.x * blockDim.x + threadIdx.x;
  const bool live = i < n;
  g1_affine_t P; P.x = Fq::zero(); P.y = Fq::zero();
  if (live) { P = load_affine(&base[i]); g_store(&table[i].x, P.x); g_store(&table[i].y, P.y); }
  const bool ident = !live || g1_affine_is_identity(P);
  bool dead = false;
  for (uint32_t w = 1; w < W; w++) {
    g1_xyzz_t acc = g1_xyzz_identity();
    fe_t z = Fq::one();
    if (!ident && !dead) {
      acc = g1_xyzz_dbl_affine<FqPs>(P);
      for (uint32_t k = 1; k < c; k++) acc = g1_xyzz_dbl<FqPs>(acc);
      z = FqPs::mul(acc.zz, acc.zzz);
      if (Fq::is_zero(z)) { dead = true; z = Fq::one(); }
    }
    fe_t total, total_r;
    const fe_t left = block_exclusive_mul_scan<false, true>(z, buf, total);
    const fe_t right = block_exclusive_mul_scan<true, true>(z, buf, total_r);
    if (threadIdx.x == 0) lds_put(inv_total, Fq::inv_sgcd(total));
    __syncthreads();
    if (dead) { P.x = Fq::zero(); P.y = Fq::zero(); }
    else if (!ident) {
      const fe_t inv = FqPs::mul(FqPs::mul(lds_get(inv_total), left), right);
      P.x = FqPs::mul(acc.x, FqPs::mul(inv, acc.zzz)); P.y = FqPs::mul(acc.y, FqPs::mul(inv, acc.zz));
    }
    if (live) { g_store(&table[w * n + i].x, P.x); g_store(&table[w * n + i].y, P.y); }
  }
}

__global__ void k_fixed_base_table(g1_affine_t *table) {
  const uint32_t d = threadIdx.x;
  g1_affine_t G; G.x = Fq::one(); G.y = Fq::dbl(Fq::one());
  g1_xyzz_t P = g1_xyzz_mul_small(g1_xyzz_from_affine(G), d);
  for (uint32_t j = 0; j < 32; j++) {
    table[j * 256 + d] = g1_xyzz_to_affine(P);
    for (int k = 0; k < 8; k++) P = g1_xyzz_dbl<FqPs>(P);
  }
}
__global__ void __launch_bounds__(256) k_fixed_base_mul(const g1_affine_t *__restrict__ table, const fe_t *__restrict__ scalars, g1_affine_t *__restrict__ out, uint64_t n) {
  const uint64_t i = (uint64_t)blockIdx.x * blockDim.x + threadIdx.x;
  if (i >= n) return;
  fe_t one_c = Fr::zero(); one_c.l[0] = 1;
  const fe_t k = FrPs::mul(g_load(&scalars[i]), one_c);
  g1_xyzz_t acc = g1_xyzz_identity();
  for (uint32_t j = 0; j < 32; j++) {
    const uint32_t d = (k.l[j >> 2] >> ((j & 3) * 8)) & 0xff;
    if (d) g1_xyzz_madd<FqPs>(acc, load_affine(&table[j * 256 + d]));
  }
  g1_affine_t r = g1_xyzz_to_affine(acc);
  g_store(&out[i].x, r.x); g_store(&out[i].y, r.y);
}
__global__ void __launch_bounds__(256) k_srs_scalars(fe_t *__restrict__ g_scal, fe_t *__restrict__ gl_scal, fe_t tau, fe_t omega, fe_t tn1_over_n, uint64_t n) {
  const uint64_t i = (uint64_t)blockIdx.x * blockDim.x + threadIdx.x;
  if (i >= n) return;
  g_store(&g_scal[i], Fr::pow_u64(tau, i));
  const fe_t wi = Fr::pow_u64(omega, i);
  const fe_t d = Fr::inv_sgcd(Fr::sub(tau, wi));
  g_store(&gl_scal[i], FrPs::mul(FrPs::mul(wi, tn1_over_n), d));
}
#endif

}
```

### scroll-prover_amd/csrc/msm_g2.hpp

```cpp
#pragma once
#include "msm.hpp"
#include "g2.hpp"

namespace zk {

#if defined(__HIPCC__)

static_assert(sizeof(g2_affine_t) == 128 && sizeof(g2_xyzz_t) == 256, "G2 record sizes (16-byte vector accesses)");

__device__ __forceinline__ g2_affine_t load_g2_affine(const g2_affine_t *p) {
  g2_affine_t r; uint32_t *w = reinterpret_cast<uint32_t *>(&r); const uint4 *q = reinterpret_cast<const uint4 *>(p);
#pragma unroll
  for (int i = 0; i < 8; i++) { const uint4 a = q[i]; w[4 * i] = a.x; w[4 * i + 1] = a.y; w[4 * i + 2] = a.z; w[4 * i + 3] = a.w; }
  return r;
}
__device__ __forceinline__ g2_xyzz_t load_g2_xyzz(const g2_xyzz_t *p) {
  g2_xyzz_t r; uint32_t *w = reinterpret_cast<uint32_t *>(&r); const uint4 *q = reinterpret_cast<const uint4 *>(p);
#pragma unroll
  for (int i = 0; i < 16; i++) { const uint4 a = q[i]; w[4 * i] = a.x; w[4 * i + 1] = a.y; w[4 * i + 2] = a.z; w[4 * i + 3] = a.w; }
  return r;
}
__device__ __forceinline__ void store_g2_xyzz(g2_xyzz_t *p, const g2_xyzz_t &v) {
  const uint32_t *w = reinterpret_cast<const uint32_t *>(&v); uint4 *q = reinterpret_cast<uint4 *>(p);
#pragma unroll
  for (int i = 0; i < 16; i++) q[i] = make_uint4(w[4 * i], w[4 * i + 1], w[4 * i + 2], w[4 * i + 3]);
}
__device__ __forceinline__ g2_xyzz_t shfl_down_g2(const g2_xyzz_t &v, uint32_t o) {
  g2_xyzz_t r; const uint32_t *s = reinterpret_cast<const uint32_t *>(&v); uint32_t *d = reinterpret_cast<uint32_t *>(&r);
#pragma unroll
  for (int i = 0; i < 64; i++) d[i] = __shfl_down(s[i], o);
  return r;
}

__global__ void __launch_bounds__(256) k_msm_g2_validate(const g2_affine_t *__restrict__ pts, uint64_t n, fe2_t b, uint32_t *__restrict__ first_bad) {
  const uint64_t stride = (uint64_t)gridDim.x * blockDim.x;
  for (uint64_t i = (uint64_t)blockIdx.x * blockDim.x + threadIdx.x; i < n; i += stride)
    if (!g2_is_on_curve_b<Fq2ps>(load_g2_affine(&pts[i]), b)) atomicMin(first_bad, (uint32_t)i);
}

struct G2Ops {
  using rec_t = g2_xyzz_t; using out_t = g2_affine_t;
  static constexpr bool QUAD = false;
  static constexpr const char *ROLE = "msm2.";
  static __device__ __forceinline__ rec_t identity() { return g2_xyzz_identity(); }
  static __device__ __forceinline__ rec_t load(const rec_t *p) { return load_g2_xyzz(p); }
  static __device__ __forceinline__ void store(rec_t *p, const rec_t &v) { store_g2_xyzz(p, v); }
  template <int Q> static __device__ __forceinline__ void add(rec_t &acc, const rec_t &o) { static_assert(Q == 1, "G2 has no quad form"); g2_xyzz_add<Fq2ps>(acc, o); }
  template <int Q> static __device__ __forceinline__ rec_t dbl(const rec_t &a) { static_assert(Q == 1, "G2 has no quad form"); return g2_xyzz_dbl<Fq2ps>(a); }
  static __device__ __forceinline__ rec_t shfl_down(const rec_t &v, uint32_t o) { return shfl_down_g2(v, o); }
  static __device__ __forceinline__ void emit(const rec_t &acc, out_t *out, int) { *out = g2_xyzz_to_affine<Fq2ps>(acc); }
};

struct G2Bases {
  using base_t = g2_affine_t;
  const g2_affine_t *__restrict__ bases;
  __device__ __forceinline__ g2_affine_t load(uint32_t e) const { return load_g2_affine(&bases[e & 0x7fffffffu]); }
  __device__ __forceinline__ void madd(g2_xyzz_t &acc, g2_affine_t p, bool neg) const {
    if (neg) p.y = Fq2ps::neg(p.y);
    g2_xyzz_madd<Fq2ps>(acc, p);
  }
};
__global__ void __launch_bounds__(256) k_msm_g2_accumulate(const g2_affine_t *__restrict__ bases, const uint32_t *__restrict__ sorted, const uint32_t *__restrict__ offsets,
                                                          uint32_t nbuckets, g2_xyzz_t *__restrict__ bucket_sums, g2_xyzz_t *__restrict__ part, int32_t *__restrict__ part_id, uint32_t seg_arg) {
  msm_segment_walk<G2Ops>(G2Bases{bases}, sorted, offsets, nbuckets, bucket_sums, part, part_id, seg_arg, blockIdx.x * blockDim.x + threadIdx.x, gridDim.x * blockDim.x);
}

#endif

}
```

Baseline: 12.56 billion G1-adds/s.

## Fuse bucket-first-point init and skip identity checks for validated SRS tables

The bucket walk now tracks a 'fresh' state, so the first point of each bucket goes straight into a dedicated init path and later points use an open madd. This removes the per-add identity test on the accumulator and the reset to identity. SRS precompute now records flags for identity points and non-canonical coordinates. When a table is clean, a trusting kernel variant skips the per-point identity-x checks and negates canonically with fewer reductions. The cost is extra template instantiations, one more branch in the walk loop, and correctness that depends on the precompute flags being right.

Result: no change. 12.60 billion G1-adds/s, median of 2 (+0.3%).

```diff
diff --git a/scroll-prover_amd/csrc/fp29.hpp b/scroll-prover_amd/csrc/fp29.hpp
--- a/scroll-prover_amd/csrc/fp29.hpp
+++ b/scroll-prover_amd/csrc/fp29.hpp
@@ -14,6 +14,10 @@
   ZK_HD static constexpr uint32_t fat29_4p(int i) { constexpr uint32_t m[9] = {0x21f3f51cu, 0x241182dau, 0x31ca8d3bu, 0x2b548b42u, 0x361765dfu, 0x2b6d0301u, 0x229b8503u, 0x397098cfu, 0xc19138u}; return m[i]; }
   ZK_HD static constexpr uint32_t fat30_8p(int i) { constexpr uint32_t m[9] = {0x43e7ea38u, 0x482305b4u, 0x43951a76u, 0x56a91685u, 0x4c2ecbbeu, 0x56da0603u, 0x45370a06u, 0x52e1319eu, 0x1832271u}; return m[i]; }
   ZK_HD static constexpr uint32_t fat30_16p(int i) { constexpr uint32_t m[9] = {0x47cfd470u, 0x50460b6au, 0x472a34eeu, 0x4d522d0cu, 0x585d977fu, 0x4db40c08u, 0x4a6e140fu, 0x45c2633eu, 0x30644e5u}; return m[i]; }
+  ZK_HD static constexpr uint32_t norm_4p(int i) { constexpr uint32_t m[9] = {0x1f3f51cu, 0x41182dbu, 0x11ca8d3cu, 0xb548b43u, 0x161765e0u, 0xb6d0302u, 0x29b8504u, 0x197098d0u, 0xc19139u}; return m[i]; }
+  ZK_HD static constexpr uint32_t norm_8p(int i) { constexpr uint32_t m[9] = {0x3e7ea38u, 0x82305b6u, 0x3951a78u, 0x16a91687u, 0xc2ecbc0u, 0x16da0605u, 0x5370a08u, 0x12e131a0u, 0x1832273u}; return m[i]; }
+  ZK_HD static constexpr uint32_t fat29_6p(int i) { constexpr uint32_t m[9] = {0x32edefaau, 0x261a4447u, 0x2aafd3d9u, 0x30fed0e4u, 0x212318cfu, 0x31238483u, 0x23e94785u, 0x3628e537u, 0x12259d5u}; return m[i]; }
+  ZK_HD static constexpr uint32_t fat29_12p(int i) { constexpr uint32_t m[9] = {0x25dbdf54u, 0x2c348890u, 0x355fa7b3u, 0x21fda1c9u, 0x224631a0u, 0x22470907u, 0x27d28f0cu, 0x2c51ca6fu, 0x244b3acu}; return m[i]; }
 };
 struct Fr29P {
   static constexpr uint32_t INV = 0xfffffffu;
@@ -205,8 +209,16 @@
     for (int i = 0; i < 9; i++) r.l[i] = borrow ? a.l[i] : d.l[i];
     return r;
   }
+  ZK_HD static uint32_t quot_est(const fe29_t &v) { return (uint32_t)(((uint64_t)(v.l[8] >> 12) * 0x15291u) >> 26); }
+  template <bool WIDE> ZK_HD static fe29_t neg_canonical(const fe29_t &v) {
+    const uint32_t k = quot_est(v) >> (WIDE ? 3 : 2);
+    fe29_t r;
+#pragma unroll
+    for (int i = 0; i < 9; i++) r.l[i] = (WIDE ? P::fat29_12p(i) : P::fat29_6p(i)) + k * (WIDE ? P::norm_8p(i) : P::norm_4p(i)) - v.l[i];
+    return carry(r);
+  }
   ZK_HD static fe29_t reduce_small(const fe29_t &v) {
-    const uint32_t q = (uint32_t)(((uint64_t)(v.l[8] >> 12) * 0x15291u) >> 26);
+    const uint32_t q = quot_est(v);
     fe29_t r; int64_t c = 0;
 #pragma unroll
     for (int i = 0; i < 9; i++) { c += (int64_t)v.l[i] - (int64_t)((uint64_t)q * P::mod(i)); r.l[i] = (i < 8) ? ((uint32_t)c & M29) : (uint32_t)c; c >>= 29; }
diff --git a/scroll-prover_amd/csrc/g1_29.hpp b/scroll-prover_amd/csrc/g1_29.hpp
--- a/scroll-prover_amd/csrc/g1_29.hpp
+++ b/scroll-prover_amd/csrc/g1_29.hpp
@@ -42,13 +42,34 @@
   if (negate) y2 = fq29_neg_loaded(y2);
   g1_xyzz29_madd_core(acc, x2, y2, negate);
 }
+ZK_HD bool g1_xyzz29_madd_open_core(g1_xyzz29_t &acc, const fe29_t &x2, const fe29_t &y2);
+ZK_HD void g1_xyzz29_first_core(g1_xyzz29_t &acc, const fe29_t &x2, const fe29_t &y2, bool y2_needs_normalise) {
+  acc.x = Fq29::reduce_small(x2); acc.y = Fq29::reduce_small(y2_needs_normalise ? Fq29::normalise(y2) : y2);
+  acc.x = Fq29::sub4(Fq29::zero(), acc.x);
+  acc.zz = Fq29::one(); acc.zzz = Fq29::one();
+}
 ZK_HD void g1_xyzz29_madd_core(g1_xyzz29_t &acc, const fe29_t &x2, const fe29_t &y2, bool y2_needs_normalise) {
-  if (g1_xyzz29_is_identity(acc)) {
-    acc.x = Fq29::reduce_small(x2); acc.y = Fq29::reduce_small(y2_needs_normalise ? Fq29::normalise(y2) : y2);
-    acc.x = Fq29::sub4(Fq29::zero(), acc.x);
+  if (g1_xyzz29_is_identity(acc)) { g1_xyzz29_first_core(acc, x2, y2, y2_needs_normalise); return; }
+  (void)g1_xyzz29_madd_open_core(acc, x2, y2);
+}
+template <bool TRUST> ZK_HD bool g1_xyzz29_first(g1_xyzz29_t &acc, const g1_affine_t &q, bool negate) {
+  if (!TRUST && g1_affine_is_identity_x(q)) { acc = g1_xyzz29_identity(); return true; }
+  const fe29_t x2 = Fq29::from_sat(q.x), y2 = Fq29::from_sat(q.y);
+  if (TRUST) {
+    acc.x = Fq29::neg_canonical<true>(x2);
+    if (negate) acc.y = Fq29::neg_canonical<false>(y2); else acc.y = Fq29::reduce_small(y2);
     acc.zz = Fq29::one(); acc.zzz = Fq29::one();
-    return;
-  }
+  } else g1_xyzz29_first_core(acc, x2, negate ? fq29_neg_loaded(y2) : y2, negate);
+  return false;
+}
+template <bool TRUST> ZK_HD bool g1_xyzz29_madd_open(g1_xyzz29_t &acc, const g1_affine_t &q, bool negate) {
+  if (!TRUST && g1_affine_is_identity_x(q)) return false;
+  const fe29_t x2 = Fq29::from_sat(q.x);
+  fe29_t y2 = Fq29::from_sat(q.y);
+  if (negate) y2 = fq29_neg_loaded(y2);
+  return g1_xyzz29_madd_open_core(acc, x2, y2);
+}
+ZK_HD bool g1_xyzz29_madd_open_core(g1_xyzz29_t &acc, const fe29_t &x2, const fe29_t &y2) {
   const fe29_t U2 = Fq29::mul_c(x2, acc.zz), S2 = Fq29::mul_c(y2, acc.zzz);
   const fe29_t Pd = Fq29::add(U2, acc.x);
   const fe29_t Rd = Fq29::sub8(S2, acc.y);
@@ -58,7 +79,7 @@
     const fe29_t one = Fq29::one();
     if (Fq29::is_zero_tight(Fq29::mul(Rd, one))) { acc = g1_xyzz29_dbl_affine(Fq29::mul(x2, one), Fq29::mul(y2, one)); acc.x = fq29_negx(acc.x); }
     else acc = g1_xyzz29_identity();
-    return;
+    return g1_xyzz29_is_identity(acc);
   }
   const fe29_t PPP = Fq29::mul_c(Pd, PP);
   const fe29_t Qn = Fq29::mul_c(acc.x, PP);
@@ -66,6 +87,7 @@
   const fe29_t T = Fq29::sub4_lazy(xn3, Qn);
   const fe29_t Y3 = Fq29::mul_sub_c(Rd, T, acc.y, PPP);
   acc.x = xn3; acc.y = Y3; acc.zz = ZZ3; acc.zzz = Fq29::mul_c(acc.zzz, PPP);
+  return false;
 }
 
 ZK_HD g1_xyzz29_t g1_xyzz29_dbl(const g1_xyzz29_t &a) {
diff --git a/scroll-prover_amd/csrc/lib_common.hpp b/scroll-prover_amd/csrc/lib_common.hpp
--- a/scroll-prover_amd/csrc/lib_common.hpp
+++ b/scroll-prover_amd/csrc/lib_common.hpp
@@ -44,7 +44,7 @@
 struct Shard { int slot = 0; uint64_t lo = 0, n = 0; g1_affine_t *dev = nullptr; bool owned = false; };
 void free_shards(std::vector<Shard> &sh);
 struct SrsMem { std::vector<Shard> sh; ~SrsMem() { free_shards(sh); } };
-struct SrsTables { std::vector<g1_affine_t *> pre; std::vector<uint64_t> stride; std::vector<int> slot; int c = 0, w = 0; ~SrsTables(); };
+struct SrsTables { std::vector<g1_affine_t *> pre; std::vector<uint64_t> stride; std::vector<int> slot; std::vector<uint32_t> flags; int c = 0, w = 0; ~SrsTables(); };
 struct Srs { uint64_t n = 0; std::shared_ptr<SrsMem> mem; std::shared_ptr<SrsTables> tab; };
 struct Buf { void *p = nullptr; size_t cap = 0; };
 struct NttPlan {
@@ -87,7 +87,7 @@
   bool profiling = false;
   std::vector<Span> spans;
   std::map<std::string, Prof> prof;
-  int last_c = 0, last_w = 0; uint64_t last_entries = 0; bool last_shared = false; int last_host_slices = 1;
+  int last_c = 0, last_w = 0; uint64_t last_entries = 0; bool last_shared = false, last_trusting = false; int last_host_slices = 1;
 };
 enum : unsigned { SYNC_COMPUTE = 1, SYNC_AUX = 2, SYNC_COPY = 4 };
 struct CtxStream { hipStream_t *s; unsigned kind; };
diff --git a/scroll-prover_amd/csrc/lib_msm.hip b/scroll-prover_amd/csrc/lib_msm.hip
--- a/scroll-prover_amd/csrc/lib_msm.hip
+++ b/scroll-prover_amd/csrc/lib_msm.hip
@@ -33,7 +33,7 @@
   return best_c;
 }
 
-struct PreTable { const g1_affine_t *table = nullptr; uint64_t row_stride = 0; int c = 0, w = 0; };
+struct PreTable { const g1_affine_t *table = nullptr; uint64_t row_stride = 0; int c = 0, w = 0; uint32_t flags = ~0u; };
 const PreTable *pre_advance(const PreTable *pre, uint64_t lo, PreTable &store) {
   if (!pre) return nullptr;
   store = *pre; if (store.table) store.table += lo;
@@ -219,7 +219,7 @@
   const bool piped = st.a != st.b;
   const Roles ws{G1Ops::ROLE, slot.id ? "#" + std::to_string(slot.id) : std::string()};
   MsmShape sh; CHK(msm_shape(n, M, pre, sh, forced));
-  const bool shared = sh.shared;
+  const bool shared = sh.shared, trusting = shared && pre->flags == 0;
   if (shared) bases = pre->table;
   const uint64_t emax = sh.emax;
   const AccPlan ap = msm_acc_plan(emax);
@@ -256,7 +256,8 @@
     {
       Scope sc("msm_accumulate", s);
       HIPCHK(hipMemsetAsync(buckets, 0, (size_t)nbuckets * sizeof(g1_xyzz29_t), s));
-      hipLaunchKernelGGL(k_msm_accumulate, dim3(acc_blocks), dim3(256), 0, s, bases, sorted, offsets, nbuckets, buckets, part, part_id, seg_arg, log2_ceil(n), shared ? pre->row_stride : (uint64_t)0);
+      auto acc_kernel = trusting ? k_msm_accumulate<true> : k_msm_accumulate<false>;
+      hipLaunchKernelGGL(acc_kernel, dim3(acc_blocks), dim3(256), 0, s, bases, sorted, offsets, nbuckets, buckets, part, part_id, seg_arg, log2_ceil(n), shared ? pre->row_stride : (uint64_t)0);
     }
     if (piped) { HIPCHK(hipEventRecord(slot.acc_done, s)); HIPCHK(hipStreamWaitEvent(st.c, slot.acc_done, 0)); }
   }
@@ -282,7 +283,7 @@
   if (piped) HIPCHK(hipEventRecord(slot.red_done, st.c));
   slot.used = true;
   HIPCHK(hipGetLastError());
-  g.last_c = (int)P.c; g.last_w = (int)P.windows; g.last_entries += emax; g.last_shared = shared;
+  g.last_c = (int)P.c; g.last_w = (int)P.windows; g.last_entries += emax; g.last_shared = shared; g.last_trusting = trusting;
   return MI355_OK;
 }
 
@@ -450,7 +451,7 @@
   HIPCHK(hipMemcpyAsync(out_host, out_dev, (size_t)M * sizeof(g2_affine_t), hipMemcpyDeviceToHost, s));
   HIPCHK(hipStreamSynchronize(s));
   resolve_spans();
-  g.last_c = (int)P.c; g.last_w = (int)P.windows; g.last_entries += sh.emax; g.last_shared = false; g.last_chunks = 1;
+  g.last_c = (int)P.c; g.last_w = (int)P.windows; g.last_entries += sh.emax; g.last_shared = false; g.last_trusting = false; g.last_chunks = 1;
   { char buf[64]; snprintf(buf, sizeof buf, " batch=%u c=%d W=%d", M, g.last_c, g.last_w); tr.done(buf); }
   return MI355_OK;
 }
@@ -631,7 +632,8 @@
   const int W = (MSM_SCALAR_BITS + c - 1) / c;
   auto tab = std::make_shared<SrsTables>();
   tab->c = c; tab->w = W;
-  tab->pre.assign(mem.sh.size(), nullptr); tab->stride.assign(mem.sh.size(), 0); tab->slot.assign(mem.sh.size(), 0);
+  tab->pre.assign(mem.sh.size(), nullptr); tab->stride.assign(mem.sh.size(), 0); tab->slot.assign(mem.sh.size(), 0); tab->flags.assign(mem.sh.size(), ~0u);
+  std::vector<uint32_t *> flags_dev(mem.sh.size(), nullptr);
   for (size_t i = 0; i < mem.sh.size(); i++) {
     const Shard &sh = mem.sh[i];
     tab->slot[i] = sh.slot;
@@ -640,10 +642,15 @@
     CHK(bind_ctx(sh.slot));
     CHK(dev_malloc((void **)&tab->pre[i], (size_t)W * cnt * sizeof(g1_affine_t), "srs_precompute (window table)"));
     tab->stride[i] = cnt;
-    hipLaunchKernelGGL(k_srs_precompute, dim3(ceil_div(cnt, 256)), dim3(256), 0, g.stream, sh.dev, tab->pre[i], cnt, (uint32_t)W, (uint32_t)c);
+    CHK(ws_get("srs.pre_flags", sizeof(uint32_t), (void **)&flags_dev[i]));
+    HIPCHK(hipMemsetAsync(flags_dev[i], 0, sizeof(uint32_t), g.stream));
+    hipLaunchKernelGGL(k_srs_precompute, dim3(ceil_div(cnt, 256)), dim3(256), 0, g.stream, sh.dev, tab->pre[i], cnt, (uint32_t)W, (uint32_t)c, flags_dev[i]);
     HIPCHK(hipGetLastError());
   }
-  for (const auto &sh : mem.sh) { CHK(bind_ctx(sh.slot)); HIPCHK(hipStreamSynchronize(g.stream)); }
+  for (size_t i = 0; i < mem.sh.size(); i++) {
+    CHK(bind_ctx(mem.sh[i].slot)); HIPCHK(hipStreamSynchronize(g.stream));
+    if (flags_dev[i]) HIPCHK(hipMemcpy(&tab->flags[i], flags_dev[i], sizeof(uint32_t), hipMemcpyDeviceToHost));
+  }
   sp->tab = tab;
   return bind_ctx(0);
   });
@@ -659,7 +666,7 @@
     const uint64_t lo = std::max(off, sh.lo), hi = std::min(off + n, sh.lo + sh.n);
     if (hi <= lo) continue;
     Piece p; p.slot = sh.slot; p.bases = sh.dev + (lo - sh.lo); p.a = lo - off; p.cnt = hi - lo;
-    if (sp->tab && sp->tab->pre[i] && hi - sh.lo <= sp->tab->stride[i]) { p.pre.table = sp->tab->pre[i] + (lo - sh.lo); p.pre.row_stride = sp->tab->stride[i]; p.pre.c = sp->tab->c; p.pre.w = sp->tab->w; }
+    if (sp->tab && sp->tab->pre[i] && hi - sh.lo <= sp->tab->stride[i]) { p.pre.table = sp->tab->pre[i] + (lo - sh.lo); p.pre.row_stride = sp->tab->stride[i]; p.pre.c = sp->tab->c; p.pre.w = sp->tab->w; p.pre.flags = sp->tab->flags[i]; }
     out.push_back(p);
   }
   if (out.empty()) { Piece p; p.slot = 0; p.bases = nullptr; p.a = 0; p.cnt = 0; out.push_back(p); }
@@ -935,7 +942,7 @@
   return guarded([&]() -> int {
   DevGuard lk(0);
   if (devices_out) *devices_out = g_last_devices; if (exchange_out) *exchange_out = g_last_exchange;
-  if (shared_tables_out) *shared_tables_out = g_ctx[0].last_shared ? 1 : 0; if (host_slices_out) *host_slices_out = g_ctx[0].last_host_slices;
+  if (shared_tables_out) *shared_tables_out = g_ctx[0].last_shared ? (g_ctx[0].last_trusting ? 2 : 1) : 0; if (host_slices_out) *host_slices_out = g_ctx[0].last_host_slices;
   return MI355_OK;
   });
 }
diff --git a/scroll-prover_amd/csrc/msm.hpp b/scroll-prover_amd/csrc/msm.hpp
--- a/scroll-prover_amd/csrc/msm.hpp
+++ b/scroll-prover_amd/csrc/msm.hpp
@@ -390,21 +390,28 @@
   uint32_t ent = sorted[start];
   uint32_t ent_next = start + 1 < end ? sorted[start + 1] : 0;
   typename B::base_t p = bases.load(ent);
+  bool fresh = true;
   for (uint32_t pos = start; pos < end; pos++) {
     typename B::base_t p_next = p;
     if (pos + 1 < end) { ent_next = sorted[pos + 1]; p_next = bases.load(ent_next); }
-    if (pos >= b_end) {
+    const auto leave_bucket = [&]() {
       if (b_start >= start) G::store(&bucket_sums[b], acc);
       else { G::store(&part[2 * (uint64_t)t], acc); id_first = (int32_t)b; }
-      acc = G::identity();
+      if constexpr (!B::FUSED_FIRST) acc = G::identity();
       b++; b_start = b_end; b_end = offsets[b + 1];
       if (pos >= b_end) {
         uint32_t l2 = b, h2 = nbuckets;
         while (h2 - l2 > 1) { const uint32_t mid = (l2 + h2) >> 1; if (offsets[mid] <= pos) l2 = mid; else h2 = mid; }
         b = l2; b_start = offsets[b]; b_end = offsets[b + 1];
       }
+    };
+    if constexpr (B::FUSED_FIRST) {
+      if (pos >= b_end || fresh) { if (pos >= b_end) leave_bucket(); fresh = bases.first(acc, p, (ent >> 31) != 0); }
+      else fresh = bases.madd_open(acc, p, (ent >> 31) != 0);
+    } else {
+      if (pos >= b_end) leave_bucket();
+      bases.madd(acc, p, (ent >> 31) != 0);
     }
-    bases.madd(acc, p, (ent >> 31) != 0);
     ent = ent_next; p = p_next;
   }
   if (b_start >= start && b_end <= end) G::store(&bucket_sums[b], acc);
@@ -412,8 +419,10 @@
   else { G::store(&part[2 * (uint64_t)t + 1], acc); id_last = (int32_t)b; }
   part_id[2 * t] = id_first; part_id[2 * t + 1] = id_last;
 }
-struct G1Bases {
+constexpr uint32_t PRE_HAS_IDENTITY = 1u, PRE_NOT_CANONICAL = 2u;
+template <bool TRUST> struct G1Bases {
   using base_t = g1_affine_t;
+  static constexpr bool FUSED_FIRST = true;
   const g1_affine_t *__restrict__ bases; uint32_t nshift; uint64_t row_stride;
   __device__ __forceinline__ const g1_affine_t *base_of(uint32_t e) const {
     const uint32_t gi = e & 0x7fffffffu;
@@ -422,15 +431,17 @@
     return &bases[(uint64_t)w * row_stride + (gi & ((1u << nshift) - 1))];
   }
   __device__ __forceinline__ g1_affine_t load(uint32_t e) const { return load_affine(base_of(e)); }
-  __device__ __forceinline__ void madd(g1_xyzz29_t &acc, const g1_affine_t &p, bool neg) const { g1_xyzz29_madd(acc, p, neg); }
+  __device__ __forceinline__ bool first(g1_xyzz29_t &acc, const g1_affine_t &p, bool neg) const { return g1_xyzz29_first<TRUST>(acc, p, neg); }
+  __device__ __forceinline__ bool madd_open(g1_xyzz29_t &acc, const g1_affine_t &p, bool neg) const { return g1_xyzz29_madd_open<TRUST>(acc, p, neg); }
 };
 struct G1AccOps : G1Ops {
   static __device__ __forceinline__ void store(rec_t *p, rec_t v) { g1_xyzz29_negx_to_plain(v); store_xyzz29(p, v); }
 };
+template <bool TRUST>
 __global__ void __launch_bounds__(256) k_msm_accumulate(const g1_affine_t *__restrict__ bases, const uint32_t *__restrict__ sorted, const uint32_t *__restrict__ offsets,
                                                         uint32_t nbuckets, g1_xyzz29_t *__restrict__ bucket_sums, g1_xyzz29_t *__restrict__ part, int32_t *__restrict__ part_id, uint32_t seg_arg,
                                                         uint32_t nshift, uint64_t row_stride) {
-  msm_segment_walk<G1AccOps>(G1Bases{bases, nshift, row_stride}, sorted, offsets, nbuckets, bucket_sums, part, part_id, seg_arg, blockIdx.x * blockDim.x + threadIdx.x, gridDim.x * blockDim.x);
+  msm_segment_walk<G1AccOps>(G1Bases<TRUST>{bases, nshift, row_stride}, sorted, offsets, nbuckets, bucket_sums, part, part_id, seg_arg, blockIdx.x * blockDim.x + threadIdx.x, gridDim.x * blockDim.x);
 }
 
 constexpr uint32_t FIXUP_SERIAL_MAX = 32, FIXUP_HUGE_MIN = 2048, FIXUP_SLICES = 64;
@@ -634,13 +645,22 @@
   if (local) atomicAdd(bad, local);
 }
 
-__global__ void __launch_bounds__(FRSCAN_THREADS) k_srs_precompute(const g1_affine_t *__restrict__ base, g1_affine_t *__restrict__ table, uint64_t n, uint32_t W, uint32_t c) {
+ZK_HD bool fq_is_canonical(const fe_t &v) {
+  for (int k = 7; k >= 0; k--) if (v.l[k] != FqP::mod(k)) return v.l[k] < FqP::mod(k);
+  return false;
+}
+__global__ void __launch_bounds__(FRSCAN_THREADS) k_srs_precompute(const g1_affine_t *__restrict__ base, g1_affine_t *__restrict__ table, uint64_t n, uint32_t W, uint32_t c,
+                                                                   uint32_t *__restrict__ flags) {
   __shared__ uint32_t buf[2 * FRSCAN_THREADS * 9];
   __shared__ uint32_t inv_total[8];
   const uint64_t i = (uint64_t)blockIdx.x * blockDim.x + threadIdx.x;
   const bool live = i < n;
   g1_affine_t P; P.x = Fq::zero(); P.y = Fq::zero();
   if (live) { P = load_affine(&base[i]); g_store(&table[i].x, P.x); g_store(&table[i].y, P.y); }
+  if (live) {
+    const uint32_t f = (g1_affine_is_identity_x(P) ? PRE_HAS_IDENTITY : 0u) | (fq_is_canonical(P.x) && fq_is_canonical(P.y) ? 0u : PRE_NOT_CANONICAL);
+    if (f) atomicOr(flags, f);
+  }
   const bool ident = !live || g1_affine_is_identity(P);
   bool dead = false;
   for (uint32_t w = 1; w < W; w++) {
@@ -663,6 +683,7 @@
       P.x = FqPs::mul(acc.x, FqPs::mul(inv, acc.zzz)); P.y = FqPs::mul(acc.y, FqPs::mul(inv, acc.zz));
     }
     if (live) { g_store(&table[w * n + i].x, P.x); g_store(&table[w * n + i].y, P.y); }
+    if (live && !ident && Fq::is_zero(P.x)) atomicOr(flags, PRE_HAS_IDENTITY);
   }
 }
 
diff --git a/scroll-prover_amd/csrc/msm_g2.hpp b/scroll-prover_amd/csrc/msm_g2.hpp
--- a/scroll-prover_amd/csrc/msm_g2.hpp
+++ b/scroll-prover_amd/csrc/msm_g2.hpp
@@ -53,6 +53,7 @@
 
 struct G2Bases {
   using base_t = g2_affine_t;
+  static constexpr bool FUSED_FIRST = false;
   const g2_affine_t *__restrict__ bases;
   __device__ __forceinline__ g2_affine_t load(uint32_t e) const { return load_g2_affine(&bases[e & 0x7fffffffu]); }
   __device__ __forceinline__ void madd(g2_xyzz_t &acc, g2_affine_t p, bool neg) const {
```
